# songxf1024/GIMS

Hardware: AMD Instinct MI355X
Metric: image-pairs/sec at 2x4096 keypoints (higher is better)
Workload: dtype bf16 MFMA attention + bf16x3 MFMA linears + f32 Sinkhorn; 1 GPU; 8 pairs/step/GPU of 2x4096 synthetic keypoints (kept 4096/4096 after AGC r=15 p=2 m=7), 256-d descriptors, 18 attentional layers (9 self + 9 cross), 100 Sinkhorn iterations, match_threshold 0.2; keypoints=4096

## Files before the change

gims_amd/csrc/agc.hip:

```cpp
#include "common.h"

#include <cstring>
#include <vector>

namespace gims {

constexpr int AGC_MAX_N = 32768;
constexpr int AGC_PK_SHIFT = 16;
constexpr uint32_t AGC_PK_MASK = 0xffffu;
constexpr int AGC_CC_LDS_N = 16384;
constexpr int AGC_NB = 16384;

struct AgcWs {
  float* dnf;
  uint16_t* dn16;
  uint16_t* S16;
  uint32_t* list;
  uint32_t* band;
  uint32_t* clist;
  uint32_t* ckey;
  uint32_t list_cap, clist_cap; int lds16;
  int32_t* cellptr;
  int32_t* cellidx;
  uint64_t* bits;
// ... 905 lines not shown
  extern __shared__ int32_t sm[];
  int32_t* list = sm;
  uint32_t* touched = (uint32_t*)(sm + w.n);
  __shared__ int wcount[17];
  const int t = threadIdx.x, lane = t & 63, wave = t >> 6;
  const int total_dir = w.counters[0];
  for (int k = t; k < (w.n + 31) / 32; k += 1024) touched[k] = 0;
  if (t == 0) wcount[16] = 0;
  __syncthreads();
  int n_added = 0;
  if (total_dir != 0 && w.n > 1) {
    for (int base = 0; base < w.n; base += 1024) {
      const int i = base + t;
      const bool iso = i < w.n && w.deg[i] == 0;
      const uint64_t m = __ballot(iso);
      if (lane == 0) wcount[wave] = __popcll(m);
      __syncthreads();
      int off = wcount[16];
      for (int q = 0; q < wave; ++q) off += wcount[q];
      if (iso) list[off + __popcll(m & ((1ull << lane) - 1))] = i;
      __syncthreads();
      if (t == 0) {
        int s = 0;
        for (int q = 0; q < 16; ++q) s += wcount[q];
        wcount[16] += s;
      }
      __syncthreads();
    }
    if (t == 0) {
      const int cnt = wcount[16];
      for (int q = 0; q < cnt; ++q) {
        const int i = list[q];
        if (touched[i >> 5] & (1u << (i & 31))) continue;
        const int j = w.nn[i];
        w.bits[(int64_t)i * w.nw + (j >> 6)] |= 1ull << (j & 63);
        w.bits[(int64_t)j * w.nw + (i >> 6)] |= 1ull << (i & 63);
        touched[j >> 5] |= 1u << (j & 31);
        ++n_added;
      }
    }
  }
  if (t == 0) info[3] = n_added;
}

__global__ __launch_bounds__(1024) void agc_scan_kernel(const AgcWs* __restrict__ ws, int mode) {
  const AgcWs& w = ws[blockIdx.y];
  const int n = w.n;
  const int32_t* deg = mode == 0 ? w.deg : (mode == 1 ? w.coff : w.degk);
  int32_t* ptr = mode == 0 ? w.ptr0 : (mode == 1 ? w.coff2 : w.indptr);
  int32_t* total_out = mode == 0 ? w.counters + 2 : (mode == 1 ? nullptr : w.info + 1);
  __shared__ int wsum[16];
  __shared__ int carry;
  const int t = threadIdx.x, lane = t & 63, wave = t >> 6;
  if (t == 0) carry = 0;
  __syncthreads();
  for (int base = 0; base < n; base += 1024) {
    const int i = base + t;
    int v = i < n ? deg[i] : 0;
    int x = v;
#pragma unroll
    for (int o = 1; o < 64; o <<= 1) {
      const int y = __shfl_up(x, o, 64);
      if (lane >= o) x += y;
    }
    if (lane == 63) wsum[wave] = x;
    __syncthreads();
    int off = carry;
    for (int q = 0; q < wave; ++q) off += wsum[q];
    if (i < n) ptr[i] = off + x - v;
    __syncthreads();
    if (t == 0) {
      int s = 0;
      for (int q = 0; q < 16; ++q) s += wsum[q];
      carry += s;
    }
    __syncthreads();
  }
  if (t == 0) {
    ptr[n] = carry;
    if (total_out) *total_out = carry;
  }
}

__global__ __launch_bounds__(256) void agc_fill_kernel(const AgcWs* __restrict__ ws, int final_pass) {
  const AgcWs& w = ws[blockIdx.y];
  const int32_t* __restrict__ ptr_by_row = final_pass ? w.indptr : w.ptr0;
  const int32_t* __restrict__ newid = final_pass ? w.newid : nullptr;
  int32_t* __restrict__ idx = final_pass ? w.indices : w.idx0;
  const int cap = final_pass ? w.max_edges_dir : w.cap;
  const int wave = threadIdx.x >> 6, lane = threadIdx.x & 63, sub = lane & 15;
  const int i = blockIdx.x * 16 + wave * 4 + (lane >> 4);
  const bool live = i < w.n && !(newid && newid[i] < 0);
  const int wpl = (w.nw + 15) / 16, k0 = sub * wpl, k1 = k0 + wpl < w.nw ? k0 + wpl : w.nw;
  int c = 0;
  if (live)
    for (int k = k0; k < k1; ++k) c += __popcll(w.bits[(int64_t)i * w.nw + k]);
  int x = c;
#pragma unroll
  for (int o = 1; o < 16; o <<= 1) {
    const int y = __shfl_up(x, o, 16);
    if (sub >= o) x += y;
  }
  if (!live) return;
  int pos = ptr_by_row[newid ? newid[i] : i] + x - c;
  for (int k = k0; k < k1; ++k) {
    uint64_t m = w.bits[(int64_t)i * w.nw + k];
    while (m) {
      const int b = __ffsll((unsigned long long)m) - 1;
      m &= m - 1;
      const int j = k * 64 + b;
      if (pos < cap) {
        idx[pos] = newid ? newid[j] : j;
        if (!final_pass) w.esrc[pos] = i;
      }
      ++pos;
    }
  }
}

template <bool GLOBAL>
__global__ __launch_bounds__(1024) void agc_cc_kernel(const AgcWs* __restrict__ ws) {
  const AgcWs& w = ws[blockIdx.y];
  const int min_size = w.min_size;
  int32_t* __restrict__ kept = w.kept;
  int32_t* info = w.info;
  extern __shared__ int32_t sm[];
  int32_t* parent = GLOBAL ? w.members : sm;
  int32_t* count = GLOBAL ? w.nnc : sm + w.n;
  auto cnt_of = [&](int x) { return __hip_atomic_load(&count[x], __ATOMIC_RELAXED, __HIP_MEMORY_SCOPE_AGENT); };
  __shared__ int wsum[16];
  __shared__ int carry[2];
  const int t = threadIdx.x, lane = t & 63, wave = t >> 6;
  const int n = w.n;
  for (int u = t; u < n; u += 1024) {
    __hip_atomic_store(&parent[u], u, __ATOMIC_RELAXED, __HIP_MEMORY_SCOPE_AGENT);
    __hip_atomic_store(&count[u], 0, __ATOMIC_RELAXED, __HIP_MEMORY_SCOPE_AGENT);
  }
  __syncthreads();
  volatile int32_t* vp = parent;
  auto find = [&](int x) {
    for (;;) {
      const int p = vp[x];
      if (p == x) return x;
      const int g = vp[p];
      if (g != p) vp[x] = g;
      x = p;
    }
  };
  {
    const int E = w.ptr0[n] < w.cap ? w.ptr0[n] : w.cap;
    for (int e0 = t; e0 < E; e0 += 4 * 1024) {
      int us[4], vs[4];
#pragma unroll
      for (int q = 0; q < 4; ++q) {
        const int e = e0 + q * 1024;
        us[q] = e < E ? w.esrc[e] : 0;
        vs[q] = e < E ? w.idx0[e] : 0;
      }
#pragma unroll
      for (int q = 0; q < 4; ++q) {
        const int u = us[q], v = vs[q];
        if (v <= u) continue;
        for (;;) {
          const int ru = find(u), rv = find(v);
          if (ru == rv) break;
          const int hi = ru > rv ? ru : rv, lo = ru > rv ? rv : ru;
          if (atomicCAS(&parent[hi], hi, lo) == hi) break;
        }
// ... 120 lines not shown
  const int C = w.counters[1];
  if (c >= C) return;
  const double cx = w.cent[2 * c], cy = w.cent[2 * c + 1];
  double bd = 1e300;
  int bj = 0x7fffffff;
  for (int j = lane; j < C; j += 64) {
    if (j == c) continue;
    const double dx = w.cent[2 * j] - cx, dy = w.cent[2 * j + 1] - cy;
    const double dd = dx * dx + dy * dy;
    if (dd < bd) { bd = dd; bj = j; }
  }
#pragma unroll
  for (int o = 32; o > 0; o >>= 1) {
    const double od = __shfl_xor(bd, o, 64);
    const int oj = __shfl_xor(bj, o, 64);
    if (od < bd || (od == bd && oj < bj)) { bd = od; bj = oj; }
  }
  if (lane == 0) w.nnc[c] = bj;
}

__global__ __launch_bounds__(256) void agc_link_kernel(const AgcWs* __restrict__ ws) {
  const AgcWs& w = ws[blockIdx.y];
  const float* __restrict__ kpts = w.kpts;
  const int32_t* __restrict__ coff = w.coff2;
  __shared__ double sd[256];
  __shared__ int sv[256], su[256];
  const int t = threadIdx.x;
  const int C = w.counters[1];
  if (C <= 1) return;
  for (int i = blockIdx.x; i < C; i += gridDim.x) {
  const int j = w.nnc[i];
  if (j < i && w.nnc[j] == i) {
    if (t == 0) { w.link[2 * i] = -1; w.link[2 * i + 1] = -1; }
    continue;
  }
  const int ai = coff[i], na = coff[i + 1] - ai;
  const int aj = coff[j], nb = coff[j + 1] - aj;
  double bd = 1e300;
  int bv = 0x7fffffff, bu = 0x7fffffff;
  const bool swap = nb > na;
  const int big0 = swap ? aj : ai, nbig = swap ? nb : na, small0 = swap ? ai : aj, nsmall = swap ? na : nb;
  for (int p = t; p < nbig; p += 256) {
    const int pb = w.members[big0 + p];
    const double bx = (double)kpts[2 * pb], by = (double)kpts[2 * pb + 1];
    for (int q = 0; q < nsmall; ++q) {
      const int ps = w.members[small0 + q];
      const double dx = bx - (double)kpts[2 * ps], dy = by - (double)kpts[2 * ps + 1];
      const double dd = dx * dx + dy * dy;
      const int v = swap ? pb : ps, u = swap ? ps : pb;
      if (dd < bd || (dd == bd && (v < bv || (v == bv && u < bu)))) { bd = dd; bv = v; bu = u; }
    }
  }
  sd[t] = bd; sv[t] = bv; su[t] = bu;
  __syncthreads();
  for (int s = 128; s > 0; s >>= 1) {
    if (t < s) {
      const double od = sd[t + s];
      const int ov = sv[t + s], ou = su[t + s];
      if (od < sd[t] || (od == sd[t] && (ov < sv[t] || (ov == sv[t] && ou < su[t])))) { sd[t] = od; sv[t] = ov; su[t] = ou; }
    }
    __syncthreads();
  }
  if (t == 0) { w.link[2 * i] = su[0]; w.link[2 * i + 1] = sv[0]; }
  __syncthreads();
  }
}

__global__ __launch_bounds__(256) void agc_link_apply_kernel(const AgcWs* __restrict__ ws) {
  const AgcWs& w = ws[blockIdx.y];
  int32_t* info = w.info;
  const int C = w.counters[1];
  if (C <= 1) { if (threadIdx.x == 0 && blockIdx.x == 0) info[5] = 0; return; }
  int added = 0;
  for (int i = blockIdx.x * 256 + threadIdx.x; i < C; i += gridDim.x * 256) {
    const int u = w.link[2 * i], v = w.link[2 * i + 1];
    if (u < 0) continue;
    atomicOr((unsigned long long*)&w.bits[(int64_t)u * w.nw + (v >> 6)], 1ull << (v & 63));
    atomicOr((unsigned long long*)&w.bits[(int64_t)v * w.nw + (u >> 6)], 1ull << (u & 63));
    ++added;
  }
  if (added) atomicAdd(&info[5], added);
}

__global__ void agc_finish_kernel(const AgcWs* __restrict__ ws, int window) {
  const AgcWs& w = ws[blockIdx.y];
  int32_t* info = w.info;
  const int max_edges_dir = w.max_edges_dir;
  info[2] = w.counters[0] / 2;
  info[6] = (int32_t)__float_as_uint(key_f32(w.sel[0]));
  info[7] = (info[1] > max_edges_dir || w.counters[0] > w.cap || w.counters[2] > w.cap) ? 1 : 0;
  if ((uint32_t)w.counters[4] > w.clist_cap) {
    info[7] = 1;
    info[2] = w.counters[4];
  }
  if (window) {
    const float thr = key_f32(w.sel[0]), vL = __uint_as_float(w.band[0]), vU = __uint_as_float(w.band[1]), eps = __uint_as_float(w.band[2]);
    if (w.counters[7] || !(thr >= vL + eps && thr <= vU - eps)) info[7] |= 2;
  } else {
    const float thr = key_f32(w.sel[0]);
    if (w.counters[7] || !(thr >= __uint_as_float(w.band[2]) && thr <= __uint_as_float(w.band[3]))) info[7] |= 2;
  }
}

__global__ __launch_bounds__(256) void agc_kept_deg_kernel(const AgcWs* __restrict__ ws) {
  const AgcWs& w = ws[blockIdx.y];
  const int u = blockIdx.x * 256 + threadIdx.x;
  if (u >= w.n) return;
  const int id = w.newid[u];
  if (id >= 0) w.degk[id] = w.deg[u];
  if (u >= w.info[0]) w.degk[u] = 0;
}

constexpr int AGC_MIN_CAP_PER_NODE = 64;

static void agc_layout(int n, int d, int max_edges_dir, bool with_s16, WsLayout& L, AgcWs& w) {
  const int nw = (n + 63) / 64, lds16 = (n + 7) & ~7;
  const int cap = max_edges_dir > n * AGC_MIN_CAP_PER_NODE ? max_edges_dir : n * AGC_MIN_CAP_PER_NODE;
  char* dn = L.take<char>((size_t)n * d * 6);
  w.dnf = (float*)dn;
  w.dn16 = dn ? (uint16_t*)(dn + (size_t)n * d * 4) : nullptr;
  const size_t list_cap = (size_t)n * (n - 1) / 2 + 64;
  w.S16 = with_s16 ? L.take<uint16_t>((size_t)n * lds16) : nullptr;
  w.clist = L.take<uint32_t>(cap);
  w.ckey = L.take<uint32_t>(cap);
  w.list = L.take<uint32_t>(list_cap);
  w.list_cap = (uint32_t)list_cap;
  w.clist_cap = (uint32_t)cap;
  w.lds16 = lds16;
  w.cellptr = L.take<int32_t>(AGC_NB + 1);
  w.cellidx = L.take<int32_t>(n);
  w.bits = L.take<uint64_t>((size_t)n * nw);
  w.hist = L.take<uint32_t>(4096);
  w.sel = L.take<uint32_t>(4);
  w.band = L.take<uint32_t>(4);
  w.deg = L.take<int32_t>(n);
  w.nn = L.take<int32_t>(n);
  w.label = L.take<int32_t>(n);
  w.alive = L.take<int32_t>(n);
  w.newid = L.take<int32_t>(n);
  w.crank = L.take<int32_t>(n);
  w.coff = L.take<int32_t>(n + 1);
  w.members = L.take<int32_t>(n);
  w.nnc = L.take<int32_t>(n);
  w.link = L.take<int32_t>((size_t)n * 2);
  w.cent = L.take<double>((size_t)n * 2);
  w.ptr0 = L.take<int32_t>(n + 1);
  w.idx0 = L.take<int32_t>(cap);
  w.esrc = L.take<int32_t>(cap);
  w.counters = L.take<int32_t>(16);
  w.coff2 = L.take<int32_t>(n + 1);
  w.degk = L.take<int32_t>(n);
  w.n = n; w.d = d; w.nw = nw; w.cap = cap;
}

static void agc_batch_layout(const gims_agc_image* images, int n_images, bool robust, WsLayout& L, AgcWs* recs) {
  L.take<AgcWs>(n_images);
  AgcWs scratch;
  for (int i = 0; i < n_images; ++i) agc_layout(images[i].n, images[i].d, images[i].max_edges_dir, robust, L, recs ? recs[i] : scratch);
}

}

static bool agc_takes_robust_flow(const gims_agc_image* images, int n_images, int flags) {
  bool robust = (flags & GIMS_AGC_ROBUST) != 0 || gims::env_int("GIMS_AGC_ROBUST", 0) != 0;
  for (int i = 0; i < n_images; ++i) robust = robust || images[i].d % gims::SW_KC != 0 || images[i].d > gims::SW_KMAX;
  return robust;
}

extern "C" size_t gims_agc_workspace_bytes(const gims_agc_image* images, int32_t n_images, int32_t flags) {
  using namespace gims;
  if (!images || n_images <= 0) return 0;
  const bool robust = agc_takes_robust_flow(images, n_images, flags);
  WsLayout L(nullptr);
  agc_batch_layout(images, n_images, robust, L, nullptr);
  return L.bytes();
}

extern "C" int32_t gims_agc_max_keypoints(void) { return gims::AGC_MAX_N; }

extern "C" int gims_agc_build(const gims_agc_image* images, int32_t n_images, const gims_agc_params* params, int32_t n_params, int32_t flags,
                              void* work, size_t work_bytes, void* stream) {
  using namespace gims;
  GIMS_CHECK_ARG(images && n_images > 0 && work, "gims_agc_build: null / empty arguments");
  GIMS_CHECK_ARG(params && (n_params == 1 || n_params == n_images), "gims_agc_build: h_params is null or n_params=%d is neither 1 nor n_images=%d",
                 n_params, n_images);
  const bool robust = agc_takes_robust_flow(images, n_images, flags);
  const char* env_shift = getenv("GIMS_AGC_WINDOW_SHIFT");
  const float window_test_shift = env_shift ? (float)atof(env_shift) : 0.f;
  for (int i = 0; i < n_images; ++i) {
    const gims_agc_image& im = images[i];
    GIMS_CHECK_ARG(im.kpts && im.desc && im.kept && im.indptr && im.indices && im.info, "gims_agc_build: image %d has a null pointer", i);
    GIMS_CHECK_ARG(im.n >= 2 && im.n <= AGC_MAX_N, "gims_agc_build: image %d: n=%d out of range [2, %d] (gims_agc_max_keypoints)", i, im.n, AGC_MAX_N);
    static_assert(AGC_MAX_N <= (1 << AGC_PK_SHIFT), "the band list packs a pair as i << 16 | j");
    GIMS_CHECK_ARG(im.d > 0 && (im.d % 32) == 0 && (im.ldd % 4) == 0, "gims_agc_build: image %d: d=%d must be a multiple of 32 (ldd %% 4 == 0)", i, im.d);
  }
  std::vector<AgcWs> hws(n_images);
  WsLayout lay(work);
  agc_batch_layout(images, n_images, robust, lay, hws.data());
  GIMS_CHECK_ARG(work_bytes >= lay.bytes(), "gims_agc_build: workspace too small (%zu bytes; gims_agc_workspace_bytes asks for %zu for the %s flow)", work_bytes,
                 lay.bytes(), robust ? "robust" : "window");
  hipStream_t s = (hipStream_t)stream;
  AgcWs* dws = (AgcWs*)work;
  int maxn = 0, maxnw = 0;
  for (int i = 0; i < n_images; ++i) {
    const gims_agc_image& im = images[i];
    AgcWs* w = &hws[i];
    w->kpts = im.kpts; w->desc = im.desc; w->ldd = im.ldd; w->kept = im.kept; w->indptr = im.indptr; w->indices = im.indices;
    w->info = im.info; w->max_edges_dir = im.max_edges_dir;
    const gims_agc_params& pm = params[n_params == 1 ? 0 : i];
    const int64_t L = (int64_t)im.n * (im.n - 1) / 2;
    int64_t k = (int64_t)(((double)L * pm.percentile) / 100.0);
    if (k >= L) k = L - 1;
    if (k < 0) k = 0;
    w->krank = k;
    double side = fabs(pm.radius) * 1.001;
    if (!(side >= 1e-3)) side = 1e-3;
    w->r2 = pm.radius * pm.radius;
    w->inv_side = 1.0 / side;
    w->min_size = pm.min_size;
    maxn = im.n > maxn ? im.n : maxn;
    maxnw = w->nw > maxnw ? w->nw : maxnw;
  }
  GIMS_LDS_ATTR((const void*)agc_cc_kernel<false>, AGC_CC_LDS_N * 8);
  GIMS_LDS_ATTR((const void*)agc_iso_seq_kernel, AGC_MAX_N * 4 + (AGC_MAX_N / 32 + 2) * 4);
  const int B = n_images;
  {
    const int rc = upload_table(hws.data(), sizeof(AgcWs) * (size_t)B, dws, s);
    if (rc != GIMS_OK) return rc;
    hipLaunchKernelGGL(agc_init_kernel, dim3(1, B), dim3(256), 0, s, dws);
  }
  const dim3 gw(cdiv(maxn, 4), B), g1(1, B);
  hipLaunchKernelGGL(agc_normalize_kernel, gw, dim3(256), 0, s, dws);
  {
    const int T = cdiv(maxn, S16_T), ntiles = T * (T + 1) / 2;
    if (robust) {
      GIMS_LDS_ATTR((const void*)agc_sim16_kernel, S16_LDS_BYTES);
      const int nparts = 8 / (((B & -B) > 8) ? 8 : (B & -B)), per_xcd = cdiv(B * nparts, 8) * cdiv(ntiles, nparts);
      const int sgrid = 8 * (per_xcd < 2 * (device_cus() / 8) ? per_xcd : 2 * (device_cus() / 8));
      int hgrid = 4096 / B;
      hgrid = hgrid < 16 ? 16 : (hgrid > 1024 ? 1024 : hgrid);
      hgrid = hgrid < maxn ? hgrid : maxn;
      hipLaunchKernelGGL(agc_sim16_kernel, dim3(sgrid), dim3(256), S16_LDS_BYTES, s, dws, B);
      hipLaunchKernelGGL(agc_band_kernel, g1, dim3(256), 0, s, dws);
      hipLaunchKernelGGL(agc_sweep16_kernel, dim3(hgrid, B), dim3(256), 0, s, dws, 1);
    } else {
      GIMS_LDS_ATTR((const void*)agc_simw_kernel<SIM_SAMPLE>, SW_LDS_BYTES);
      GIMS_LDS_ATTR((const void*)agc_simw_kernel<SIM_COLLECT>, SW_LDS_BYTES);
      const int wgrid = 8 * 2 * (device_cus() / 8);
      hipLaunchKernelGGL(agc_simw_kernel<SIM_SAMPLE>, dim3(wgrid), dim3(256), SW_LDS_BYTES, s, dws, B);
      hipLaunchKernelGGL(agc_window_kernel, g1, dim3(256), 0, s, dws, window_test_shift);
      hipLaunchKernelGGL(agc_simw_kernel<SIM_COLLECT>, dim3(wgrid), dim3(256), SW_LDS_BYTES, s, dws, B);
    }
    GIMS_LDS_ATTR((const void*)agc_grid_kernel, AGC_NB * 4);
    hipLaunchKernelGGL(agc_grid_kernel, g1, dim3(1024), AGC_NB * 4, s, dws);
    hipLaunchKernelGGL(agc_radius_grid_kernel, dim3(cdiv(maxn, 32), B), dim3(288), 0, s, dws);
    hipLaunchKernelGGL(agc_exact_kernel, dim3(8 * 4 * (device_cus() / 8)), dim3(256), 0, s, dws, B, robust ? 0 : 1);
    const int lgrid = 1024 / B < 4 ? 4 : (1024 / B > 64 ? 64 : 1024 / B);
    hipLaunchKernelGGL(agc_hist_kernel, dim3(lgrid, B), dim3(256), 0, s, dws, 20, 12);
    hipLaunchKernelGGL(agc_pick_kernel, g1, dim3(256), 0, s, dws, 20, 12);
    hipLaunchKernelGGL(agc_hist_kernel, dim3(lgrid, B), dim3(256), 0, s, dws, 8, 12);
    hipLaunchKernelGGL(agc_pick_kernel, g1, dim3(256), 0, s, dws, 8, 12);
    hipLaunchKernelGGL(agc_hist_kernel, dim3(lgrid, B), dim3(256), 0, s, dws, 0, 8);
    hipLaunchKernelGGL(agc_pick_kernel, g1, dim3(256), 0, s, dws, 0, 8);
  }
  hipLaunchKernelGGL(agc_apply_kernel, dim3(16, B), dim3(256), 0, s, dws);
  hipLaunchKernelGGL(agc_deg_kernel, dim3(cdiv(maxn, 16), B), dim3(256), 0, s, dws, 1);
  hipLaunchKernelGGL(agc_iso_nn_kernel, gw, dim3(256), 0, s, dws);
  const size_t iso_lds = (size_t)maxn * 4 + ((size_t)(maxn + 31) / 32 + 1) * 4;
  hipLaunchKernelGGL(agc_iso_seq_kernel, g1, dim3(1024), iso_lds, s, dws);
  hipLaunchKernelGGL(agc_deg_kernel, dim3(cdiv(maxn, 16), B), dim3(256), 0, s, dws, 0);
  hipLaunchKernelGGL(agc_scan_kernel, g1, dim3(1024), 0, s, dws, 0);
  hipLaunchKernelGGL(agc_fill_kernel, dim3(cdiv(maxn, 16), B), dim3(256), 0, s, dws, 0);
  if (maxn <= AGC_CC_LDS_N) hipLaunchKernelGGL(agc_cc_kernel<false>, g1, dim3(1024), (size_t)maxn * 8, s, dws);
  else hipLaunchKernelGGL(agc_cc_kernel<true>, g1, dim3(1024), 0, s, dws);
  hipLaunchKernelGGL(agc_scan_kernel, g1, dim3(1024), 0, s, dws, 1);
  if (maxn <= 16384) hipLaunchKernelGGL(agc_members_kernel<4>, dim3(32, B), dim3(256), 0, s, dws);
  else hipLaunchKernelGGL(agc_members_kernel<8>, dim3(32, B), dim3(512), 0, s, dws);
  hipLaunchKernelGGL(agc_nnc_kernel, gw, dim3(256), 0, s, dws);
  hipLaunchKernelGGL(agc_link_kernel, dim3(maxn < 256 ? maxn : 256, B), dim3(256), 0, s, dws);
  hipLaunchKernelGGL(agc_link_apply_kernel, dim3(cdiv(maxn, 256), B), dim3(256), 0, s, dws);
  hipLaunchKernelGGL(agc_deg_kernel, dim3(cdiv(maxn, 16), B), dim3(256), 0, s, dws, 0);
  hipLaunchKernelGGL(agc_kept_deg_kernel, dim3(cdiv(maxn, 256), B), dim3(256), 0, s, dws);
  hipLaunchKernelGGL(agc_scan_kernel, g1, dim3(1024), 0, s, dws, 2);
  hipLaunchKernelGGL(agc_fill_kernel, dim3(cdiv(maxn, 16), B), dim3(256), 0, s, dws, 1);
  hipLaunchKernelGGL(agc_finish_kernel, g1, dim3(1), 0, s, dws, robust ? 0 : 1);
  GIMS_LAUNCH_CHECK();
  return GIMS_OK;
}
```

gims_amd/csrc/common.h:

```cpp
#pragma once
#include <hip/hip_runtime.h>
#include <stdint.h>
#include <stdio.h>
#include <stdlib.h>

#include "../../include/gims_hip.h"

namespace gims {

void set_error(const char* fmt, ...);

#define GIMS_CHECK_ARG(cond, ...)                    \
  do {                                               \
    if (!(cond)) {                                   \
      ::gims::set_error(__VA_ARGS__);                \
      return GIMS_EINVAL;                            \
    }                                                \
  } while (0)

#define GIMS_HIP(call)                                                                     \
  do {                                                                                     \
    hipError_t e_ = (call);                                                                \
    if (e_ != hipSuccess) {                                                                \
      ::gims::set_error("%s failed: %s (%s:%d)", #call, hipGetErrorString(e_), __FILE__, __LINE__); \
// ... 48 lines not shown
#pragma unroll
  for (int o = 32; o > 0; o >>= 1) v = fmaxf(v, __shfl_xor(v, o, 64));
  return v;
}
__device__ __forceinline__ double wave_sum_f64(double v) {
#pragma unroll
  for (int o = 32; o > 0; o >>= 1) v += __shfl_xor(v, o, 64);
  return v;
}

__device__ __forceinline__ uint32_t f32_key(float x) {
  uint32_t u = __float_as_uint(x);
  return (u & 0x80000000u) ? ~u : (u | 0x80000000u);
}
__device__ __forceinline__ float key_f32(uint32_t k) {
  uint32_t u = (k & 0x80000000u) ? (k & 0x7fffffffu) : ~k;
  return __uint_as_float(u);
}

__device__ __forceinline__ void ot_raise_status(float* status, float code) {
  __hip_atomic_fetch_max((int*)status, __float_as_int(code), __ATOMIC_RELAXED, __HIP_MEMORY_SCOPE_AGENT);
}

__device__ __forceinline__ bool attn_guard_fires(const gims_attn_guard& g) {
  const unsigned long long* st = (const unsigned long long*)g.stat;
  const int lane = threadIdx.x & 63, nw = 4 * (g.n_heads + 1);
  const unsigned long long v = lane < nw ? __builtin_nontemporal_load(st + lane) : 0ull;
  bool mine = false;
  if (g.kind == GIMS_GUARD_PEAKED) {
    const unsigned long long cnt = __shfl(v, (lane & ~3) + 1, 64), tail = __shfl(v, (lane & ~3) + 3, 64);
    const unsigned long long mx = __shfl(v, (lane & ~3) + 2, 64);
    if ((lane & 3) == 0 && lane < 4 * g.n_heads) {
      if (cnt != 0) {
        const double mean = (double)v / (double)cnt / 16777216.0, tl = (double)tail / (double)cnt;
        mine = mean > g.mean_thr || tl > g.tail_thr;
      }
      mine = mine || (g.max_thr > 0.0 && (double)mx / 16777216.0 >= g.max_thr);
    }
  } else if (lane >= 4 * g.n_heads && lane < 4 * g.n_heads + 3) {
    mine = !((double)__uint_as_float((uint32_t)v) <= g.range_limit);
  }
  return __ballot(mine) != 0ull;
}

static inline int cdiv(int64_t a, int64_t b) { return (int)((a + b - 1) / b); }

static inline size_t al256(size_t x) { return (x + 255) & ~(size_t)255; }
struct WsLayout {
  char* base;
  size_t off = 0;
  explicit WsLayout(void* b) : base((char*)b) {}
  template <typename T> T* take(size_t count) { const size_t o = off; off += al256(sizeof(T) * count); return base ? (T*)(base + o) : nullptr; }
  size_t bytes() const { return off; }
};
static inline int env_int(const char* name, int dflt) { const char* e = getenv(name); return e ? atoi(e) : dflt; }
static inline bool guard_walk_enabled() { return env_int("GIMS_GUARD_WALK", 1) != 0; }

int upload_table(const void* host, size_t bytes, void* dev, hipStream_t stream);
int lds_attr(const void* fn, int bytes);
void* device_once(const char* key, size_t bytes, const void* init);
void* pinned_once(const char* key, size_t bytes);
int current_device();
int device_cus();
void count_linear_launch(int kind);
int linear_x6_batch_launch(const gims_linear_args* dev_args, int count, int max_m, int max_n, hipStream_t s);
int split_spl3_launch(const float* src, int64_t lds, uint16_t* dst, int64_t ldd, int64_t rows, int k, hipStream_t s);

int mlp_fused_launch(const gims_linear_args& a, hipStream_t s);

int sift_describe_aux(const gims_aux_args& x, hipStream_t st);
int diou_nms_aux(const gims_aux_args& x, hipStream_t st);
int assemble_rows_aux(const gims_aux_args& x, hipStream_t st);
int build_tracks_aux(const gims_aux_args& x, hipStream_t st);
int triangulate_tracks_aux(const gims_aux_args& x, hipStream_t st);
int resect_images_aux(const gims_aux_args& x, hipStream_t st);
int bundle_adjust_aux(const gims_aux_args& x, hipStream_t st);
int bundle_adjust_pcg_aux(const gims_aux_args& x, hipStream_t st);
int bundle_adjust_focal_aux(const gims_aux_args& x, hipStream_t st);
int select_pairs_aux(const gims_aux_args& x, hipStream_t st);

struct OtR2Host { const float* z; int64_t ld; int n, m; float* u; float* v; float* status; float norm, log_mu_bin, log_nu_bin; };
struct OtR2Plan { bool ok; int nx, nc, ppg, ngroups; size_t bytes; };
OtR2Plan ot_res2_plan(const OtR2Host* pr, int np, int iters);
int ot_res2_run(const OtR2Plan& P, const OtR2Host* hp, int np, float alpha, int iters, int init_inside, char* base, hipStream_t s);

}
```

gims_amd/csrc/misc.hip:

```cpp
#include "common.h"

#include <stdarg.h>
#include <string.h>

#include <map>
#include <mutex>
#include <string>
#include <utility>

namespace gims {

static thread_local char g_err[512] = "";
void set_error(const char* fmt, ...) {
  va_list ap;
  va_start(ap, fmt);
  vsnprintf(g_err, sizeof(g_err), fmt, ap);
  va_end(ap);
}

int current_device() {
  int dev = 0;
  if (hipGetDevice(&dev) != hipSuccess) dev = 0;
  return dev;
}

int device_cus() {
  int n = 0;
  if (hipDeviceGetAttribute(&n, hipDeviceAttributeMultiprocessorCount, current_device()) != hipSuccess || n < 8) n = 8;
  return n;
}

static std::mutex g_once_mu;

int lds_attr(const void* fn, int bytes) {
  static std::map<std::pair<const void*, int>, int> done;
  const int dev = current_device();
  std::lock_guard<std::mutex> lock(g_once_mu);
  int& have = done[std::make_pair(fn, dev)];
  if (have >= bytes) return GIMS_OK;
  GIMS_HIP(hipFuncSetAttribute(fn, hipFuncAttributeMaxDynamicSharedMemorySize, bytes));
  have = bytes;
  return GIMS_OK;
}

void* device_once(const char* key, size_t bytes, const void* init) {
  static std::map<std::pair<std::string, int>, void*> bufs;
  const int dev = current_device();
  std::lock_guard<std::mutex> lock(g_once_mu);
  void*& p = bufs[std::make_pair(std::string(key), dev)];
  if (p) return p;
  void* d = nullptr;
  if (hipMalloc(&d, bytes) != hipSuccess) return nullptr;
  if ((init ? hipMemcpy(d, init, bytes, hipMemcpyHostToDevice) : hipMemset(d, 0, bytes)) != hipSuccess) { (void)hipFree(d); return nullptr; }
  p = d;
  return p;
}

void* pinned_once(const char* key, size_t bytes) {
  static std::map<std::pair<std::string, int>, void*> bufs;
  const int dev = current_device();
  std::lock_guard<std::mutex> lock(g_once_mu);
  void*& p = bufs[std::make_pair(std::string(key), dev)];
  if (p) return p;
  void* h = nullptr;
  if (hipHostMalloc(&h, bytes) != hipSuccess) return nullptr;
  memset(h, 0, bytes);
  p = h;
  return p;
}

struct Blob4K { uint4 v[248]; };
__global__ void put_blob_kernel(Blob4K blob, uint4* __restrict__ dst, int n16) {
  if ((int)threadIdx.x < n16) dst[threadIdx.x] = blob.v[threadIdx.x];
}

int upload_table(const void* host, size_t bytes, void* dev, hipStream_t stream) {
  const char* h = (const char*)host;
  char* d = (char*)dev;
  for (size_t off = 0; off < bytes; off += sizeof(Blob4K)) {
    Blob4K blob;
    const size_t n = bytes - off < sizeof(Blob4K) ? bytes - off : sizeof(Blob4K);
    memcpy(&blob, h + off, n);
    hipLaunchKernelGGL(put_blob_kernel, dim3(1), dim3(256), 0, stream, blob, (uint4*)(d + off), (int)((n + 15) / 16));
  }
  GIMS_LAUNCH_CHECK();
  return GIMS_OK;
}

}

extern "C" int gims_upload_table(const void* host, int64_t bytes, void* dev, void* stream) {
  using namespace gims;
  GIMS_CHECK_ARG(host && dev && bytes >= 0 && bytes <= (1 << 20) && ((uintptr_t)dev & 15) == 0, "gims_upload_table: bad arguments");
  if (bytes == 0) return GIMS_OK;
  return upload_table(host, (size_t)bytes, dev, (hipStream_t)stream);
}

namespace gims {
template <bool RELU>
__global__ __launch_bounds__(256) void kenc_first_kernel(const float* __restrict__ kpts, const float* __restrict__ norm3,
                                                         const int32_t* __restrict__ seg, const float* __restrict__ w1,
                                                         const float* __restrict__ b1, int c1, float* __restrict__ out,
                                                         int64_t n, int n_img) {
  const int64_t idx = (int64_t)blockIdx.x * blockDim.x + threadIdx.x;
  const int64_t row = idx / c1;
  const int ch = (int)(idx - row * c1);
  if (row >= n) return;
  int img;
  if (n_img > 0) {
    int lo = 0, hi = n_img - 1;
    while (lo < hi) {
      const int mid = (lo + hi + 1) >> 1;
      if ((int64_t)seg[mid] <= row) lo = mid; else hi = mid - 1;
    }
    img = lo;
  } else {
    img = seg[row];
  }
  const float* nm = norm3 + 3 * img;
  const float x = (kpts[2 * row] - nm[0]) / nm[2];
  const float y = (kpts[2 * row + 1] - nm[1]) / nm[2];
  float v = fmaf(w1[2 * ch + 1], y, fmaf(w1[2 * ch], x, b1[ch]));
  out[row * c1 + ch] = RELU ? fmaxf(v, 0.f) : v;
}

__global__ __launch_bounds__(256) void layernorm_act_kernel(const float* __restrict__ x, int64_t ldx, int64_t rows, int c,
                                                            const float* __restrict__ a2, const float* __restrict__ b2, float eps, int act,
                                                            float* __restrict__ out, int64_t ldo, uint16_t* __restrict__ out_hi,
                                                            uint16_t* __restrict__ out_lo, int64_t ld_split) {
  const int64_t row = (int64_t)blockIdx.x * 4 + (threadIdx.x >> 6);
  const int lane = threadIdx.x & 63;
  if (row >= rows) return;
  const float* xr = x + row * ldx;
  float v[8];
  float s = 0.f;
#pragma unroll
  for (int k = 0; k < 8; ++k) {
    const int ch = lane + 64 * k;
    v[k] = ch < c ? xr[ch] : 0.f;
    s += v[k];
  }
  const float mean = wave_sum(s) / (float)c;
  float q = 0.f;
#pragma unroll
  for (int k = 0; k < 8; ++k) {
    const float d = lane + 64 * k < c ? v[k] - mean : 0.f;
    q += d * d;
  }
  const float sd = sqrtf(wave_sum(q) / (float)(c - 1));
  const float inv = 1.f / (sd + eps);
#pragma unroll
  for (int k = 0; k < 8; ++k) {
    const int ch = lane + 64 * k;
    if (ch < c) {
      float y = a2[ch] * ((v[k] - mean) * inv) + b2[ch];
      if (act == GIMS_ACT_RELU) y = fmaxf(y, 0.f);
      if (out) out[row * ldo + ch] = y;
      if (out_hi) {
        const uint16_t h = f2bf(y);
        out_hi[row * ld_split + spl_col(ch)] = h;
        out_lo[row * ld_split + spl_col(ch)] = f2bf(y - bf2f(h));
      }
    }
  }
}

__global__ __launch_bounds__(256) void sage_mean_kernel(const float* __restrict__ h, int64_t ldh,
                                                        const int32_t* __restrict__ indptr,
                                                        const int32_t* __restrict__ indices, int n, int c,
                                                        float* __restrict__ out, int64_t ldo,
                                                        uint16_t* __restrict__ out_spl, int64_t ld_spl) {
  const int wave = threadIdx.x >> 6, lane = threadIdx.x & 63;
  const int node = blockIdx.x * 4 + wave;
  if (node >= n) return;
  const int beg = indptr[node], end = indptr[node + 1];
  for (int q0 = 0; 4 * q0 < c; q0 += 64) {
    const int q = q0 + lane;
    const bool act = 4 * q < c;
    const int qq = act ? q : 0;
    float4 s = make_float4(0.f, 0.f, 0.f, 0.f);
    for (int e0 = beg; e0 < end; e0 += 64) {
      const int cnt = end - e0 < 64 ? end - e0 : 64;
      const int mine = lane < cnt ? indices[e0 + lane] : 0;
      int e = 0;
      for (; e + 4 <= cnt; e += 4) {
        const float4 x0 = *(const float4*)(h + (int64_t)__shfl(mine, e, 64) * ldh + 4 * qq);
        const float4 x1 = *(const float4*)(h + (int64_t)__shfl(mine, e + 1, 64) * ldh + 4 * qq);
        const float4 x2 = *(const float4*)(h + (int64_t)__shfl(mine, e + 2, 64) * ldh + 4 * qq);
        const float4 x3 = *(const float4*)(h + (int64_t)__shfl(mine, e + 3, 64) * ldh + 4 * qq);
        s.x += x0.x; s.y += x0.y; s.z += x0.z; s.w += x0.w;
        s.x += x1.x; s.y += x1.y; s.z += x1.z; s.w += x1.w;
        s.x += x2.x; s.y += x2.y; s.z += x2.z; s.w += x2.w;
        s.x += x3.x; s.y += x3.y; s.z += x3.z; s.w += x3.w;
      }
      for (; e < cnt; ++e) {
        const float4 x = *(const float4*)(h + (int64_t)__shfl(mine, e, 64) * ldh + 4 * qq);
        s.x += x.x; s.y += x.y; s.z += x.z; s.w += x.w;
      }
    }
    if (!act) continue;
    if (end > beg) {
      const float d = (float)(end - beg);
      s.x /= d; s.y /= d; s.z /= d; s.w /= d;
    }
    if (out) *(float4*)(out + (int64_t)node * ldo + 4 * q) = s;
    if (out_spl) {
      const uint32_t h01 = pack_bf2(s.x, s.y), h23 = pack_bf2(s.z, s.w);
      const uint32_t l01 = pack_bf2(s.x - __uint_as_float(h01 << 16), s.y - __uint_as_float(h01 & 0xffff0000u));
      const uint32_t l23 = pack_bf2(s.z - __uint_as_float(h23 << 16), s.w - __uint_as_float(h23 & 0xffff0000u));
      uint16_t* o = out_spl + (int64_t)node * ld_spl + spl_col(4 * q);
      *(uint2*)o = make_uint2(h01, h23);
      *(uint2*)(o + 32) = make_uint2(l01, l23);
    }
  }
}

__global__ __launch_bounds__(256) void gather_rows_kernel(const float* __restrict__ src, int64_t lds,
                                                          const int32_t* __restrict__ idx, int n, int c,
                                                          float* __restrict__ dst, int64_t ldd) {
  const int wave = threadIdx.x >> 6, lane = threadIdx.x & 63;
  const int row = blockIdx.x * 4 + wave;
  if (row >= n) return;
  const float* s = src + (int64_t)idx[row] * lds;
  float* d = dst + (int64_t)row * ldd;
  for (int j = lane; j < c; j += 64) d[j] = s[j];
}

__global__ __launch_bounds__(256) void pack_graphs_kernel(const gims_pack_image* __restrict__ imgs, int d,
                                                          float* __restrict__ feat, int64_t ldf,
                                                          float* __restrict__ kpts_out, float* __restrict__ score_out,
                                                          int32_t* __restrict__ seg, int32_t* __restrict__ indptr_out,
                                                          int32_t* __restrict__ indices_out, int n_rows_total,
                                                          int n_edges_total) {
  const gims_pack_image im = imgs[blockIdx.y];
  const int wave = threadIdx.x >> 6, lane = threadIdx.x & 63;
  for (int r = blockIdx.x * 4 + wave; r < im.n_kept; r += gridDim.x * 4) {
    const int src = im.kept[r];
    const float4* s = (const float4*)(im.desc + (int64_t)src * im.ldd);
    float4* o = (float4*)(feat + (int64_t)(im.row_off + r) * ldf);
    for (int q = lane; 4 * q < d; q += 64) o[q] = s[q];
    if (lane == 0) {
      kpts_out[2 * (im.row_off + r)] = im.kpts[2 * src];
      kpts_out[2 * (im.row_off + r) + 1] = im.kpts[2 * src + 1];
      if (score_out && im.score) score_out[im.row_off + r] = im.score[src];
      seg[im.row_off + r] = blockIdx.y;
      if (im.src_row) im.src_row[im.row_off + r] = im.in_off + src;
      indptr_out[im.row_off + r] = im.indptr[r] + im.edge_off;
    }
  }
  for (int e = blockIdx.x * 256 + threadIdx.x; e < im.n_edges; e += gridDim.x * 256)
    indices_out[im.edge_off + e] = im.indices[e] + im.row_off;
  if (blockIdx.x == 0 && blockIdx.y == 0 && threadIdx.x == 0) indptr_out[n_rows_total] = n_edges_total;
}

__global__ __launch_bounds__(256) void ingest_kernel(const gims_ingest_image* __restrict__ imgs, int d,
                                                     float* __restrict__ desc_out, int64_t ldo,
                                                     float* __restrict__ kpts_out, float* __restrict__ score_out) {
  __shared__ float tile[64][65];
  const gims_ingest_image im = imgs[blockIdx.z];
  const int n0 = blockIdx.x * 64, d0 = blockIdx.y * 64;
  if (n0 >= im.n) return;
  const int c = threadIdx.x & 63, r4 = threadIdx.x >> 6;
#pragma unroll
  for (int i = 0; i < 16; ++i) {
    const int r = 4 * i + r4;
    const int n = n0 + c;
    tile[r][c] = (d0 + r < d && n < im.n) ? im.desc[(int64_t)(d0 + r) * im.ldd + n] : 0.f;
  }
  __syncthreads();
#pragma unroll
  for (int i = 0; i < 16; ++i) {
    const int r = 4 * i + r4;
    const int n = n0 + r;
    if (n < im.n && d0 + c < d) desc_out[(int64_t)(im.row_off + n) * ldo + d0 + c] = tile[c][r];
  }
  if (blockIdx.y == 0 && threadIdx.x < 64) {
    const int n = n0 + threadIdx.x;
    if (n < im.n) {
      kpts_out[2 * (im.row_off + n)] = im.kpts[2 * n];
      kpts_out[2 * (im.row_off + n) + 1] = im.kpts[2 * n + 1];
      if (score_out) score_out[im.row_off + n] = im.score ? im.score[n] : 0.f;
    }
  }
}

}

extern "C" int gims_ingest_images(const gims_ingest_image* dev_images, int32_t n_images, int32_t max_n, int32_t d,
                                  float* desc_out, int64_t ldo, float* kpts_out, float* score_out, void* stream) {
  using namespace gims;
  GIMS_CHECK_ARG(dev_images && n_images > 0 && max_n > 0 && d > 0 && desc_out && kpts_out, "gims_ingest_images: bad arguments");
  hipLaunchKernelGGL(ingest_kernel, dim3(cdiv(max_n, 64), cdiv(d, 64), n_images), dim3(256), 0, (hipStream_t)stream,
                     dev_images, d, desc_out, ldo, kpts_out, score_out);
  GIMS_LAUNCH_CHECK();
  return GIMS_OK;
}

extern "C" int gims_pack_graphs(const gims_pack_image* dev_images, int32_t n_images, int32_t max_kept, int32_t max_edges,
                                int32_t d, float* feat, int64_t ldf, float* kpts_out, float* score_out, int32_t* seg,
                                int32_t* indptr_out, int32_t* indices_out, int32_t n_rows_total, int32_t n_edges_total,
                                void* stream) {
  using namespace gims;
  GIMS_CHECK_ARG(dev_images && n_images > 0 && feat && kpts_out && seg && indptr_out && indices_out, "gims_pack_graphs: null pointer");
  GIMS_CHECK_ARG((d % 4) == 0 && (ldf % 4) == 0, "gims_pack_graphs: d / ldf must be multiples of 4");
  int gx = cdiv(max_kept, 4);
  const int ge = cdiv(max_edges, 256);
  gx = gx > ge ? gx : ge;
  if (gx < 1) gx = 1;
  if (gx > 1024) gx = 1024;
  hipLaunchKernelGGL(pack_graphs_kernel, dim3(gx, n_images), dim3(256), 0, (hipStream_t)stream, dev_images, d, feat, ldf,
                     kpts_out, score_out, seg, indptr_out, indices_out, n_rows_total, n_edges_total);
  GIMS_LAUNCH_CHECK();
  return GIMS_OK;
}

static int kenc_first_images(const float* kpts, const float* norm3, const int32_t* starts, const float* w1, const float* b1, int32_t c1,
                             float* out, int64_t n, int32_t n_img, hipStream_t stream) {
  using namespace gims;
  GIMS_CHECK_ARG(kpts && norm3 && starts && w1 && b1 && out && c1 > 0 && n >= 0, "gims_run_ops: GIMS_AUX_KENC_FIRST: bad arguments");
  if (n == 0) return GIMS_OK;
  hipLaunchKernelGGL(kenc_first_kernel<true>, dim3(cdiv(n * c1, 256)), dim3(256), 0, stream, kpts, norm3, starts, w1, b1, c1, out, n, n_img);
  GIMS_LAUNCH_CHECK();
  return GIMS_OK;
}

extern "C" int gims_run_ops(const gims_op* ops, int32_t n_ops, void* stream) {
  using namespace gims;
  GIMS_CHECK_ARG(ops && n_ops >= 0, "gims_run_ops: bad arguments");
  for (int i = 0; i < n_ops; ++i) {
    int rc;
    if (ops[i].kind == GIMS_OP_LINEAR) {
      rc = gims_linear(&ops[i].u.lin, stream);
    } else if (ops[i].kind == GIMS_OP_ATTENTION) {
      rc = gims_attention(&ops[i].u.att, stream);
    } else if (ops[i].kind == GIMS_OP_MLP) {
      rc = mlp_fused_launch(ops[i].u.lin, (hipStream_t)stream);
    } else if (ops[i].kind == GIMS_OP_AUX) {
      const gims_aux_args& x = ops[i].u.aux;
      if (x.fn == GIMS_AUX_SPLIT_SPL32)
        rc = gims_split_spl32((const float*)x.p[0], x.i[0], (uint16_t*)x.p[1], x.i[1], x.i[2], (int32_t)x.i[3], stream);
      else if (x.fn == GIMS_AUX_SAGE_MEAN_SPLIT)
        rc = gims_sage_mean_split((const float*)x.p[0], x.i[0], (const int32_t*)x.p[1], (const int32_t*)x.p[2], (int32_t)x.i[1], (int32_t)x.i[2],
                                  (uint16_t*)x.p[3], x.i[3], stream);
      else if (x.fn == GIMS_AUX_KENC_FIRST && x.i[2] > 0)
        rc = kenc_first_images((const float*)x.p[0], (const float*)x.p[1], (const int32_t*)x.p[2], (const float*)x.p[3], (const float*)x.p[4],
                               (int32_t)x.i[0], (float*)x.p[5], x.i[1], (int32_t)x.i[2], (hipStream_t)stream);
      else if (x.fn == GIMS_AUX_KENC_FIRST)
        rc = gims_kenc_first((const float*)x.p[0], (const float*)x.p[1], (const int32_t*)x.p[2], (const float*)x.p[3], (const float*)x.p[4],
                             (int32_t)x.i[0], (float*)x.p[5], x.i[1], stream);
      else if (x.fn == GIMS_AUX_SAGE_MEAN)
        rc = gims_sage_mean((const float*)x.p[0], x.i[0], (const int32_t*)x.p[1], (const int32_t*)x.p[2], (int32_t)x.i[1], (int32_t)x.i[2],
                            (float*)x.p[3], x.i[3], stream);
      else if (x.fn == GIMS_AUX_KENC_FIRST_LINEAR)
        rc = gims_kenc_first_linear((const float*)x.p[0], (const float*)x.p[1], (const int32_t*)x.p[2], (const float*)x.p[3], (const float*)x.p[4],
                                    (int32_t)x.i[0], (float*)x.p[5], x.i[1], stream);
      else if (x.fn == GIMS_AUX_LAYERNORM_ACT)
        rc = gims_layernorm_act((const float*)x.p[0], x.i[0], x.i[1], (int32_t)x.i[2], (const float*)x.p[1], (const float*)x.p[2], x.f[0], (int32_t)x.i[3],
                                (float*)x.p[3], x.i[4], (uint16_t*)x.p[4], (uint16_t*)x.p[5], x.i[5], stream);
      else if (x.fn == GIMS_AUX_SIFT_DESCRIBE)
        rc = sift_describe_aux(x, (hipStream_t)stream);
      else if (x.fn == GIMS_AUX_DIOU_NMS)
        rc = diou_nms_aux(x, (hipStream_t)stream);
      else if (x.fn == GIMS_AUX_ASSEMBLE_ROWS)
        rc = assemble_rows_aux(x, (hipStream_t)stream);
      else if (x.fn == GIMS_AUX_BUILD_TRACKS)
        rc = build_tracks_aux(x, (hipStream_t)stream);
      else if (x.fn == GIMS_AUX_TRIANGULATE_TRACKS)
        rc = triangulate_tracks_aux(x, (hipStream_t)stream);
      else if (x.fn == GIMS_AUX_RESECT_IMAGES)
        rc = resect_images_aux(x, (hipStream_t)stream);
      else if (x.fn == GIMS_AUX_BUNDLE_ADJUST)
        rc = bundle_adjust_aux(x, (hipStream_t)stream);
      else if (x.fn == GIMS_AUX_BUNDLE_ADJUST_PCG)
        rc = bundle_adjust_pcg_aux(x, (hipStream_t)stream);
      else if (x.fn == GIMS_AUX_BUNDLE_ADJUST_FOCAL)
        rc = bundle_adjust_focal_aux(x, (hipStream_t)stream);
      else if (x.fn == GIMS_AUX_SELECT_PAIRS)
        rc = select_pairs_aux(x, (hipStream_t)stream);
      else
        GIMS_CHECK_ARG(false, "gims_run_ops: op %d: unknown auxiliary function %d", i, x.fn);
    } else {
      GIMS_CHECK_ARG(false, "gims_run_ops: op %d has unknown kind %d", i, ops[i].kind);
    }
    if (rc != GIMS_OK) return rc;
  }
  return GIMS_OK;
}

extern "C" int gims_run_ops_timed(const gims_op* ops, int32_t n_ops, void* stream, void* const* events) {
  using namespace gims;
  GIMS_CHECK_ARG(ops && n_ops >= 0 && events, "gims_run_ops_timed: bad arguments");
  GIMS_HIP(hipEventRecord((hipEvent_t)events[0], (hipStream_t)stream));
  for (int i = 0; i < n_ops; ++i) {
    const int rc = gims_run_ops(ops + i, 1, stream);
    if (rc != GIMS_OK) return rc;
    GIMS_HIP(hipEventRecord((hipEvent_t)events[i + 1], (hipStream_t)stream));
  }
  return GIMS_OK;
}

extern "C" int gims_events_create(int32_t n, void** events_out) {
  using namespace gims;
  GIMS_CHECK_ARG(n > 0 && events_out, "gims_events_create: bad arguments");
  for (int i = 0; i < n; ++i) {
    hipEvent_t e = nullptr;
    const hipError_t rc = hipEventCreate(&e);
    if (rc != hipSuccess) {
      for (int j = 0; j < i; ++j) (void)hipEventDestroy((hipEvent_t)events_out[j]);
      GIMS_HIP(rc);
    }
    events_out[i] = (void*)e;
  }
  return GIMS_OK;
}

extern "C" int gims_events_elapsed(void* const* events, int32_t n, float* ms_out) {
  using namespace gims;
  GIMS_CHECK_ARG(events && n > 1 && ms_out, "gims_events_elapsed: bad arguments");
  for (int i = 0; i + 1 < n; ++i) GIMS_HIP(hipEventElapsedTime(&ms_out[i], (hipEvent_t)events[i], (hipEvent_t)events[i + 1]));
  return GIMS_OK;
}

extern "C" int gims_events_destroy(void* const* events, int32_t n) {
  using namespace gims;
  GIMS_CHECK_ARG(events && n >= 0, "gims_events_destroy: bad arguments");
  for (int i = 0; i < n; ++i)
    if (events[i]) GIMS_HIP(hipEventDestroy((hipEvent_t)events[i]));
  return GIMS_OK;
}

extern "C" int gims_ops_graph_create(const gims_op* ops, int32_t n_ops, void* stream, void** graph_exec_out) {
  using namespace gims;
  GIMS_CHECK_ARG(ops && n_ops > 0 && graph_exec_out && stream, "gims_ops_graph_create: bad arguments (a non-default stream is required)");
  hipStream_t s = (hipStream_t)stream;
  GIMS_HIP(hipStreamBeginCapture(s, hipStreamCaptureModeThreadLocal));
  const int rc = gims_run_ops(ops, n_ops, stream);
  hipGraph_t graph = nullptr;
  const hipError_t e = hipStreamEndCapture(s, &graph);
  if (rc != GIMS_OK) { if (graph) (void)hipGraphDestroy(graph); return rc; }
  GIMS_HIP(e);
  hipGraphExec_t exec = nullptr;
  const hipError_t e2 = hipGraphInstantiate(&exec, graph, nullptr, nullptr, 0);
  (void)hipGraphDestroy(graph);
  GIMS_HIP(e2);
  *graph_exec_out = (void*)exec;
  return GIMS_OK;
}

extern "C" int gims_ops_graph_launch(void* graph_exec, void* stream) {
  using namespace gims;
  GIMS_CHECK_ARG(graph_exec, "gims_ops_graph_launch: null graph");
  GIMS_HIP(hipGraphLaunch((hipGraphExec_t)graph_exec, (hipStream_t)stream));
  return GIMS_OK;
}

extern "C" int gims_ops_graph_destroy(void* graph_exec) {
  using namespace gims;
  if (graph_exec) GIMS_HIP(hipGraphExecDestroy((hipGraphExec_t)graph_exec));
  return GIMS_OK;
}

extern "C" int gims_abi_version(void) { return GIMS_ABI_VERSION; }
extern "C" const char* gims_last_error(void) { return gims::g_err; }

extern "C" int gims_kenc_first(const float* kpts, const float* norm3, const int32_t* seg_of_row, const float* w1,
                               const float* b1, int32_t c1, float* out, int64_t n, void* stream) {
  using namespace gims;
  GIMS_CHECK_ARG(kpts && norm3 && seg_of_row && w1 && b1 && out && c1 > 0 && n >= 0, "gims_kenc_first: bad arguments");
  if (n == 0) return GIMS_OK;
  hipLaunchKernelGGL(kenc_first_kernel<true>, dim3(cdiv(n * c1, 256)), dim3(256), 0, (hipStream_t)stream, kpts, norm3,
                     seg_of_row, w1, b1, c1, out, n, 0);
  GIMS_LAUNCH_CHECK();
  return GIMS_OK;
}

extern "C" int gims_kenc_first_linear(const float* kpts, const float* norm3, const int32_t* seg_of_row, const float* w1,
                                      const float* b1, int32_t c1, float* out, int64_t n, void* stream) {
  using namespace gims;
  GIMS_CHECK_ARG(kpts && norm3 && seg_of_row && w1 && b1 && out && c1 > 0 && n >= 0, "gims_kenc_first_linear: bad arguments");
  if (n == 0) return GIMS_OK;
  hipLaunchKernelGGL(kenc_first_kernel<false>, dim3(cdiv(n * c1, 256)), dim3(256), 0, (hipStream_t)stream, kpts, norm3,
                     seg_of_row, w1, b1, c1, out, n, 0);
  GIMS_LAUNCH_CHECK();
  return GIMS_OK;
}

extern "C" int gims_layernorm_act(const float* x, int64_t ldx, int64_t rows, int32_t c, const float* a2, const float* b2, float eps,
                                  int32_t act, float* out, int64_t ldo, uint16_t* out_hi, uint16_t* out_lo, int64_t ld_split,
                                  void* stream) {
  using namespace gims;
  GIMS_CHECK_ARG(x && a2 && b2 && (out || out_hi) && rows >= 0 && c >= 2 && c <= 512, "gims_layernorm_act: bad arguments (2 <= c <= 512)");
  GIMS_CHECK_ARG((out_hi == nullptr) == (out_lo == nullptr), "gims_layernorm_act: out_hi and out_lo come together");
  GIMS_CHECK_ARG(ldx >= c && (!out || ldo >= c) && (!out_hi || ld_split >= 2 * (int64_t)((c + 31) / 32 * 32)),
                 "gims_layernorm_act: pitch below the row width (ldx, ldo >= c; SPL32 pitch >= 2 * c rounded up to 32 channels)");
  if (rows == 0) return GIMS_OK;
  hipLaunchKernelGGL(layernorm_act_kernel, dim3((unsigned)cdiv(rows, 4)), dim3(256), 0, (hipStream_t)stream, x, ldx, rows, c, a2, b2, eps,
                     act, out, ldo, out_hi, out_lo, ld_split);
  GIMS_LAUNCH_CHECK();
  return GIMS_OK;
}

extern "C" int gims_sage_mean(const float* h, int64_t ldh, const int32_t* indptr, const int32_t* indices, int32_t n,
                              int32_t c, float* out, int64_t ldo, void* stream) {
  using namespace gims;
  GIMS_CHECK_ARG(h && indptr && indices && out && n >= 0, "gims_sage_mean: bad arguments");
  GIMS_CHECK_ARG((c % 4) == 0 && (ldh % 4) == 0 && (ldo % 4) == 0, "gims_sage_mean: c / ld must be multiples of 4");
  if (n == 0) return GIMS_OK;
  hipLaunchKernelGGL(sage_mean_kernel, dim3(cdiv(n, 4)), dim3(256), 0, (hipStream_t)stream, h, ldh, indptr, indices, n, c,
                     out, ldo, (uint16_t*)nullptr, (int64_t)0);
  GIMS_LAUNCH_CHECK();
  return GIMS_OK;
}

extern "C" int gims_sage_mean_split(const float* h, int64_t ldh, const int32_t* indptr, const int32_t* indices, int32_t n,
                                    int32_t c, uint16_t* out_spl, int64_t ld_spl, void* stream) {
  using namespace gims;
  GIMS_CHECK_ARG(h && indptr && indices && out_spl && n >= 0, "gims_sage_mean_split: bad arguments");
  GIMS_CHECK_ARG((c % 4) == 0 && (ldh % 4) == 0 && (ld_spl % 4) == 0 && ld_spl >= 2 * (int64_t)((c + 31) / 32 * 32) && ((uintptr_t)out_spl & 7) == 0,
                 "gims_sage_mean_split: c / ldh multiples of 4, SPL32 output pitch >= 2 * c rounded up to 32 channels");
  if (n == 0) return GIMS_OK;
  hipLaunchKernelGGL(sage_mean_kernel, dim3(cdiv(n, 4)), dim3(256), 0, (hipStream_t)stream, h, ldh, indptr, indices, n, c,
                     (float*)nullptr, (int64_t)0, out_spl, ld_spl);
  GIMS_LAUNCH_CHECK();
  return GIMS_OK;
}

__global__ __launch_bounds__(256) void pair_stats_kernel(const int64_t* __restrict__ matches0, const float* __restrict__ scores0,
                                                         const int32_t* __restrict__ tab, float* __restrict__ out) {
  const int p = blockIdx.x, t = threadIdx.x;
  const int n0 = tab[4 * p + 1], off = tab[4 * p + 3];
  __shared__ float ssum[256];
  __shared__ int scnt[256];
  float s = 0.f;
  int c = 0;
  for (int i = t; i < n0; i += 256)
    if (matches0[off + i] >= 0) { s += scores0[off + i]; ++c; }
  ssum[t] = s;
  scnt[t] = c;
  __syncthreads();
  for (int o = 128; o > 0; o >>= 1) {
    if (t < o) { ssum[t] += ssum[t + o]; scnt[t] += scnt[t + o]; }
    __syncthreads();
  }
  if (t == 0) {
    float* r = out + 5 * p;
    r[0] = (float)tab[4 * p]; r[1] = (float)n0; r[2] = (float)tab[4 * p + 2];
    r[3] = (float)scnt[0]; r[4] = ssum[0] / fmaxf((float)scnt[0], 1.f);
  }
}

extern "C" int gims_pair_stats(const int64_t* matches0, const float* scores0, const int32_t* table, int32_t n_pairs, float* out,
                               void* stream) {
  using namespace gims;
  GIMS_CHECK_ARG(matches0 && scores0 && table && out && n_pairs >= 0, "gims_pair_stats: bad arguments");
  if (n_pairs == 0) return GIMS_OK;
  hipLaunchKernelGGL(pair_stats_kernel, dim3(n_pairs), dim3(256), 0, (hipStream_t)stream, matches0, scores0, table, out);
  GIMS_LAUNCH_CHECK();
  return GIMS_OK;
}

extern "C" int gims_gather_rows(const float* src, int64_t lds, const int32_t* idx, int32_t n, int32_t c, float* dst,
                                int64_t ldd, void* stream) {
  using namespace gims;
  GIMS_CHECK_ARG(src && idx && dst && n >= 0 && c > 0, "gims_gather_rows: bad arguments");
  GIMS_CHECK_ARG(lds >= c && ldd >= c, "gims_gather_rows: pitch below the row width");
// ... 6 lines not shown
```

gims_amd/csrc/sinkhorn.hip:

```cpp
#include "common.h"

#include <stdio.h>
#include <stdlib.h>
#include <string.h>

#include <map>
#include <mutex>
#include <type_traits>
#include <vector>

namespace gims {

constexpr int OT_R = 8;

struct OtDev {
  const float* z; int64_t ld; int n, m;
  float* u; float* v;
  float* partial;
  float* cbest_val; int* cbest_idx;
  float* max0; int* idx0;
  float* max1; int* idx1;
  int64_t* matches0; int64_t* matches1; float* mscores0; float* mscores1;
  float* status;
  int G;
// ... 1023 lines not shown
  const int rows = ot_instance(cpt, [](auto inst) { return decltype(inst)::R; });
  const int total = threads >= 1024 ? 256 : (threads >= 512 ? 512 : 1024);
  int cap = total / (np > 0 ? np : 1);
  if (cap < 4) cap = 4;
  int g = (n + rows - 1) / rows;
  return g < cap ? g : cap;
}
static void ot_fill_common(const gims_ot_problem& q, float& norm, float& log_mu_bin, float& log_nu_bin) {
  const float ms = (float)q.n, ns = (float)q.m;
  norm = -logf(ms + ns);
  log_mu_bin = logf(ns) + norm;
  log_nu_bin = logf(ms) + norm;
}

struct OtWs { int threads, cpt, maxn, maxm, maxG; OtR2Plan plan2; char* onchip; };
static OtWs ot_layout(const gims_ot_problem* pr, int np, int flags, WsLayout& L, OtDev* recs) {
  OtWs w{};
  ot_launch_shape(pr, np, w.threads, w.cpt, w.maxn, w.maxm);
  L.take<OtDev>(np);
  for (int i = 0; i < np; ++i) {
    const gims_ot_problem& q = pr[i];
    OtDev d{};
    d.G = ot_G(q.n, np, w.threads, w.cpt);
    w.maxG = d.G > w.maxG ? d.G : w.maxG;
    d.partial = L.take<float>((size_t)d.G * (q.m + 1));
    d.cbest_val = L.take<float>((size_t)d.G * q.m);
    d.cbest_idx = L.take<int>((size_t)d.G * q.m);
    d.max0 = L.take<float>(q.n);
    d.idx0 = L.take<int>(q.n);
    d.max1 = L.take<float>(q.m);
    d.idx1 = L.take<int>(q.m);
    if (!recs) continue;
    d.z = q.scores; d.ld = q.ld; d.n = q.n; d.m = q.m;
    d.u = q.uv; d.v = q.uv + q.n + 1; d.status = q.uv + q.n + 1 + q.m + 1;
    d.matches0 = q.matches0; d.matches1 = q.matches1; d.mscores0 = q.mscores0; d.mscores1 = q.mscores1;
    ot_fill_common(q, d.norm, d.log_mu_bin, d.log_nu_bin);
    recs[i] = d;
  }
  w.plan2 = ot_res2_choose(pr, np, 1, flags);
  w.onchip = L.take<char>(w.plan2.bytes);
  return w;
}

static void ot_streamed_iteration(const OtWs& w, const OtDev* dp, int np, float alpha, int rescue, int hist_slot, hipStream_t s) {
  const dim3 gi(w.maxG, np), gc(cdiv(w.maxm + 1, 64), np), bt(w.threads);
  ot_instance(w.cpt, [&](auto inst) { using I = decltype(inst); hipLaunchKernelGGL((ot_iter_kernel<I::CPT, I::R>), gi, bt, 0, s, dp, alpha, rescue); });
  hipLaunchKernelGGL(ot_colreduce_kernel, gc, dim3(1024), 0, s, dp, hist_slot, rescue);
}

}

extern "C" int gims_sinkhorn_plan(const gims_ot_problem* pr, int32_t np, int32_t iters, int32_t flags) {
  using namespace gims;
  if (!pr || np <= 0) return 0;
  const OtR2Plan p2 = ot_res2_choose(pr, np, iters, flags);
  return p2.ok ? p2.ngroups : 0;
}

extern "C" int gims_sinkhorn_match(const gims_ot_problem* pr, int32_t np, float alpha, int32_t iters, float match_threshold, void* work,
                                   size_t work_bytes, int32_t flags, void* stream) {
  using namespace gims;
  hipStream_t s = (hipStream_t)stream;
  GIMS_CHECK_ARG(pr && np > 0 && work, "gims_sinkhorn_match: null / empty arguments");
  GIMS_CHECK_ARG(iters >= 0, "gims_sinkhorn_match: iters < 0");
  for (int i = 0; i < np; ++i) {
    const gims_ot_problem& q = pr[i];
    GIMS_CHECK_ARG(q.n > 0 && q.m > 0 && q.scores && q.uv && q.matches0 && q.matches1 && q.mscores0 && q.mscores1,
                   "gims_sinkhorn_match: problem %d has empty shape or null pointer", i);
    GIMS_CHECK_ARG((q.ld % 4) == 0 && (((uintptr_t)q.scores) & 15) == 0, "gims_sinkhorn_match: scores must be 16-byte aligned with ld %% 4 == 0");
  }
  std::vector<OtDev> hprob(np);
  WsLayout L(work);
  const OtWs w = ot_layout(pr, np, flags, L, hprob.data());
  GIMS_CHECK_ARG(work_bytes >= L.bytes(), "gims_sinkhorn_match: workspace too small (%zu < %zu)", work_bytes, L.bytes());
  GIMS_CHECK_ARG(w.cpt <= 8, "gims_sinkhorn_match: m=%d too large (max 32768 columns: a thread of the streamed kernels owns at most 8 column quads)", w.maxm);
  const int threads = w.threads, cpt = w.cpt, maxn = w.maxn, maxm = w.maxm;
  {
    const int rc = upload_table(hprob.data(), sizeof(OtDev) * (size_t)np, work, s);
    if (rc != GIMS_OK) return rc;
  }
  const OtDev* dp = (const OtDev*)work;
  const bool onchip = w.plan2.ok && iters >= 1;
  const int init_inside = onchip && env_int("GIMS_OT_R2_INIT", 1) ? 1 : 0;
  if (init_inside) hipLaunchKernelGGL(ot_status0_kernel, dim3(cdiv(np, 256)), dim3(256), 0, s, dp, np);
  else hipLaunchKernelGGL(ot_init_kernel, dim3(cdiv(maxn, 4), np), dim3(256), 0, s, dp, alpha, iters == 0 ? 1 : 0, 0);
  const dim3 gi(w.maxG, np);
  if (onchip) {
    std::vector<OtR2Host> h2(np);
    for (int i = 0; i < np; ++i) {
      const OtDev& d = hprob[i];
      h2[i] = OtR2Host{d.z, d.ld, d.n, d.m, d.u, d.v, d.status, d.norm, d.log_mu_bin, d.log_nu_bin};
    }
    const int rc = ot_res2_run(w.plan2, h2.data(), np, alpha, iters, init_inside, w.onchip, s);
    if (rc != GIMS_OK) return rc;
    const int force_fail = env_int("GIMS_OT_FORCE_FAIL", 0);
    if (force_fail) hipLaunchKernelGGL(ot_poison_kernel, dim3(np), dim3(256), 0, s, dp);
    OtRescueState* rs = ot_rescue_state();
    if (!rs) { set_error("gims_sinkhorn_match: no rescue state on this device"); return GIMS_EHIP; }
    const int mode = env_int("GIMS_OT_RESCUE", -1);
    bool marginal;
    {
      std::lock_guard<std::mutex> lock(g_rescue_mu);
      rs->calls += 1;
      if (*rs->h_count != rs->seen) { rs->seen = *rs->h_count; rs->last_giveup_call = rs->calls; }
      marginal = mode == 1 || (mode != 0 && rs->calls - rs->last_giveup_call <= OT_MARGINAL_CALLS);
    }
    if (marginal) {
      hipLaunchKernelGGL(ot_rescue_begin_kernel, dim3(cdiv(np, 256)), dim3(256), 0, s, dp, np, rs->d_count);
      hipLaunchKernelGGL(ot_init_kernel, dim3(cdiv(maxn, 4), np), dim3(256), 0, s, dp, alpha, 0, 1);
      for (int it = 0; it < iters; ++it) ot_streamed_iteration(w, dp, np, alpha, 1, -1, s);
      hipLaunchKernelGGL(ot_rescue_end_kernel, dim3(cdiv(np, 256)), dim3(256), 0, s, dp, np);
    }
    hipLaunchKernelGGL(ot_rescue_kernel, dim3(np), dim3(1024), 0, s, dp, alpha, iters, 0, rs->d_count);
    if (hipEventQuery(rs->ev) != hipErrorNotReady) {
      GIMS_HIP(hipMemcpyAsync((void*)rs->h_count, rs->d_count, sizeof(int), hipMemcpyDeviceToHost, s));
      GIMS_HIP(hipEventRecord(rs->ev, s));
    }
  } else {
    for (int it = 0; it < iters; ++it) ot_streamed_iteration(w, dp, np, alpha, 0, -1, s);
  }
  ot_instance(cpt, [&](auto inst) { using I = decltype(inst); hipLaunchKernelGGL((ot_select_kernel<I::CPT, I::RS>), gi, dim3(threads), 0, s, dp); });
  hipLaunchKernelGGL(ot_colbest_kernel, dim3(cdiv(maxm, 32), np), dim3(256), 0, s, dp);
  const int mx = maxn > maxm ? maxn : maxm;
  hipLaunchKernelGGL(ot_mutual_kernel, dim3(cdiv(mx, 256), np), dim3(256), 0, s, dp, match_threshold);
  GIMS_LAUNCH_CHECK();
  return GIMS_OK;
}

extern "C" size_t gims_sinkhorn_workspace_bytes(const gims_ot_problem* pr, int32_t np) {
  using namespace gims;
  if (!pr || np <= 0) return 0;
  WsLayout L(nullptr);
  ot_layout(pr, np, 0, L, nullptr);
  return L.bytes();
}

extern "C" int64_t gims_sinkhorn_rescues(void) {
  using namespace gims;
  OtRescueState* rs = ot_rescue_state();
  int n = 0;
  if (!rs || hipDeviceSynchronize() != hipSuccess || hipMemcpy(&n, rs->d_count, sizeof(int), hipMemcpyDeviceToHost) != hipSuccess) {
    set_error("gims_sinkhorn_rescues: the counter of the current device could not be read");
    return -1;
  }
  return n;
}

extern "C" int gims_ot_matrix(const float* scores, int64_t ld, int32_t n, int32_t m, float alpha, const float* uv,
                              float* out, void* stream) {
  using namespace gims;
  GIMS_CHECK_ARG(scores && uv && out && n > 0 && m > 0, "gims_ot_matrix: bad arguments");
  hipLaunchKernelGGL(ot_matrix_kernel, dim3(cdiv(m + 1, 256), n + 1), dim3(256), 0, (hipStream_t)stream, scores, ld, n, m,
                     alpha, uv, out);
  GIMS_LAUNCH_CHECK();
  return GIMS_OK;
}

extern "C" int gims_train_loss(const gims_loss_pair* dev_pairs, int32_t n_pairs, const int64_t* gt, int32_t n_gt, float alpha,
                               float pos_weight, float neg_weight, float* loss_vec, int32_t* tag, float* out3, void* stream) {
  using namespace gims;
  GIMS_CHECK_ARG(dev_pairs && n_pairs > 0 && n_pairs <= 1024 && out3 && n_gt >= 0 && (n_gt == 0 || (gt && loss_vec && tag)),
                 "gims_train_loss: bad arguments (1 <= n_pairs <= 1024)");
  if (n_gt > 0) hipLaunchKernelGGL(train_loss_gather_kernel, dim3(cdiv(n_gt, 256)), dim3(256), 0, (hipStream_t)stream, dev_pairs, n_pairs, gt, n_gt, alpha,
                                   loss_vec, tag);
  hipLaunchKernelGGL(train_loss_reduce_kernel, dim3(1), dim3(1024), 0, (hipStream_t)stream, loss_vec, tag, n_gt, n_pairs, pos_weight, neg_weight, out3);
  GIMS_LAUNCH_CHECK();
  return GIMS_OK;
}

extern "C" size_t gims_sinkhorn_history_floats(int32_t n, int32_t m, int32_t iters) {
  return (size_t)(iters + 1) * (size_t)(n + m + 2);
}

extern "C" int gims_sinkhorn_history(const gims_ot_problem* pr, int32_t np, float alpha, int32_t iters, float* const* h_hist, void* work,
                                     size_t work_bytes, void* stream) {
  using namespace gims;
// ... 132 lines not shown
```

gims_amd/csrc/sinkhorn2d.hip:

```cpp
#include "common.h"

#include <stdlib.h>

#include <map>
#include <mutex>
#include <type_traits>
#include <vector>

namespace gims {

struct OtR2Block { int prob, xr, cc, pad; };
struct OtR2Dev {
  const float* z; int64_t ld; int n, m;
  float* u; float* v; float* status;
  float norm, log_mu_bin, log_nu_bin;
  float mu, mu_bin, nu_bin;
  int nx, nc;
  int rb, cb;
  int rbf, rbs;
  float* rpart;
  float* fbuf;
  float* cpart;
  float* mpart;
  int* placement;
  int* rflag;
};
struct OtR2Args {
  const OtR2Dev* probs;
  int p0, pcount, nx, nc;
  float alpha; int iters, refresh, wt_local;
  int init_inside;
  unsigned long long* prof;
};

constexpr int R2_FLAG_ITERS = 1024;
constexpr int R2_CSEG = 132;
constexpr int R2_NT = 512;
struct R2L {
  static constexpr int NW = R2_NT / 64;
  static constexpr int K = 16 * R2_NT * 4;
  static constexpr int NXMAX = 4;
  static constexpr int ROWST = 1028, FACS = 1160, GVEC = 132, COLRED = NW * 128, PB = 2 * R2_NT + 4, PR = 132, CSST = 132;
  static constexpr int XRD = 4 * R2_CSEG;
  static constexpr int OWN = 2 * 132 + 2 * 132;
  static constexpr int FLOATS = K + ROWST + FACS + GVEC + COLRED + PB + PR + CSST + XRD + 16 + OWN;
};

typedef float r2f2 __attribute__((ext_vector_type(2)));

__device__ __forceinline__ void r2_st4_wt(float* p, f32x4 v) { asm volatile("global_store_dwordx4 %0, %1, off sc1" ::"v"(p), "v"(v) : "memory"); }
__device__ __forceinline__ void r2_st4_plain(float* p, f32x4 v) { asm volatile("global_store_dwordx4 %0, %1, off" ::"v"(p), "v"(v) : "memory"); }
__device__ __forceinline__ void r2_ld4_issue(f32x4& v, const float* p) { asm volatile("global_load_dwordx4 %0, %1, off sc1" : "=&v"(v) : "v"(p) : "memory"); }
__device__ __forceinline__ void r2_ld4_wait(f32x4& a) { asm volatile("s_waitcnt vmcnt(0)" : "+v"(a)::"memory"); }
__device__ __forceinline__ void r2_swap16(float& x, float& y) { asm("s_nop 1\n\tv_permlane16_swap_b32 %0, %1" : "+v"(x), "+v"(y)); }
__device__ __forceinline__ void r2_swap32(float& x, float& y) { asm("s_nop 1\n\tv_permlane32_swap_b32 %0, %1" : "+v"(x), "+v"(y)); }
template <int CTRL>
__device__ __forceinline__ float r2_dpp_max(float x) {
  return fmaxf(x, __builtin_bit_cast(float, __builtin_amdgcn_update_dpp(0, __builtin_bit_cast(int, x), CTRL, 0xf, 0xf, true)));
}
template <int CTRL>
__device__ __forceinline__ float r2_dpp_add(float x) {
  return x + __builtin_bit_cast(float, __builtin_amdgcn_update_dpp(0, __builtin_bit_cast(int, x), CTRL, 0xf, 0xf, true));
}
__device__ __forceinline__ float r2_sum8(float x) {
  x = r2_dpp_add<0xB1>(x);
  x = r2_dpp_add<0x4E>(x);
  return r2_dpp_add<0x141>(x);
}

template <bool PROF>
__global__ __launch_bounds__(R2_NT, 1) void ot_res2_kernel(OtR2Args a) {
#pragma clang fp contract(off)
  using L = R2L;
  constexpr int NT = R2_NT;
  __shared__ int fail_flag;
  __shared__ unsigned long long prof_acc[8];
  unsigned long long prof_t = 0;
  auto stamp = [&](int phase) {
    if (PROF && threadIdx.x == 0) {
      const unsigned long long now = __builtin_readcyclecounter();
      if (phase >= 0) prof_acc[phase] += now - prof_t;
      prof_t = now;
    }
  };
  if (PROF && threadIdx.x < 8) prof_acc[threadIdx.x] = 0;
// ... 668 lines not shown
    float* rpart = L.take<float>((size_t)P.nx * P.nc * rbs);
    float* fbuf = L.take<float>((size_t)P.nx * 2 * rbs);
    float* cpart = L.take<float>((size_t)2 * P.nx * P.nc * R2_CSEG);
    float* mpart = L.take<float>((size_t)P.nx * P.nc * rbs);
    if (!recs) continue;
    const OtR2Host& d = pr[i];
    OtR2Dev q{};
    q.z = d.z; q.ld = d.ld; q.n = d.n; q.m = d.m; q.u = d.u; q.v = d.v; q.status = d.status;
    q.norm = d.norm; q.log_mu_bin = d.log_mu_bin; q.log_nu_bin = d.log_nu_bin;
    q.mu = (float)exp((double)d.norm); q.mu_bin = (float)exp((double)d.log_mu_bin); q.nu_bin = (float)exp((double)d.log_nu_bin);
    q.nx = P.nx; q.nc = P.nc; q.rb = rb; q.cb = r2_up4(cdiv(d.m, P.nc)); q.rbf = rbf; q.rbs = rbs;
    q.rpart = rpart; q.fbuf = fbuf; q.cpart = cpart; q.mpart = mpart;
    q.placement = w.dplace;
    recs[i] = q;
  }
  w.ex1 = L.bytes();
  for (int i = 0; i < np; ++i) {
    int* rflag = L.take<int>(R2_FLAG_ITERS + 8);
    if (recs) recs[i].rflag = rflag;
  }
  w.rf1 = L.bytes();
  L.take<OtR2Block>((size_t)512 * P.ngroups);
  return w;
}

static OtR2Plan plan_class(const OtR2Host* pr, int np, int iters) {
  OtR2Plan P{};
  if (iters < 1 || np < 1) return P;
  int nx = 0, nc = 0;
  if (!r2_geom(pr[0].n, pr[0].m, nx, nc)) return P;
  for (int i = 1; i < np; ++i) {
    int nxi = 0, nci = 0;
    if (!r2_geom(pr[i].n, pr[i].m, nxi, nci) || nxi != nx || nci != nc) return P;
  }
  const int units = 8 * (32 / nc);
  if (nx > units) return P;
  P.nx = nx; P.nc = nc;
  P.ppg = units / nx;
  P.ppg = P.ppg < np ? P.ppg : np;
  P.ngroups = cdiv(np, P.ppg);
  if (P.ngroups > 64) return P;
  for (int i = 0; i < np; ++i) {
    const int rb = cdiv(pr[i].n, nx);
    if (r2_up4(cdiv(rb + 1, nc)) > R2_FOLD || rb > r2_rbmax() || r2_up4(cdiv(pr[i].m, nc)) > 128) return P;
  }
  WsLayout L(nullptr);
  r2_layout(P, pr, np, L, nullptr);
  P.bytes = L.bytes();
  P.ok = true;
  return P;
}

static std::vector<std::vector<int>> r2_classes(const OtR2Host* pr, int np) {
  std::vector<std::vector<int>> out;
  std::vector<int> keys;
  for (int i = 0; i < np; ++i) {
    const int k = r2_class_key(pr[i]);
    size_t c = 0;
    while (c < keys.size() && keys[c] != k) ++c;
    if (c == keys.size()) { keys.push_back(k); out.emplace_back(); }
    out[c].push_back(i);
  }
  return out;
}

OtR2Plan ot_res2_plan(const OtR2Host* pr, int np, int iters) {
  OtR2Plan P{};
  if (iters < 1 || np < 1) return P;
  P.ok = true;
  for (const std::vector<int>& cls : r2_classes(pr, np)) {
    std::vector<OtR2Host> sub;
    for (int i : cls) sub.push_back(pr[i]);
    const OtR2Plan c = plan_class(sub.data(), (int)sub.size(), iters);
    if (!c.ok) return OtR2Plan{};
    P.nx = c.nx > P.nx ? c.nx : P.nx;
    P.nc = c.nc > P.nc ? c.nc : P.nc;
    P.ppg = c.ppg > P.ppg ? c.ppg : P.ppg;
    P.ngroups += c.ngroups;
    P.bytes += al256(c.bytes);
  }
  return P;
}

static int run_class(const OtR2Plan& P, const OtR2Host* hp, int np, float alpha, int iters, int init_inside, char* base, hipStream_t s);

struct R2State { int resident_ok, wt_local; volatile int* h_place; hipEvent_t place_ev; };
static R2State* r2_state(const void* kernel, int threads, int blocks, size_t lds) {
  static std::mutex mu;
  static std::map<int, R2State> states;
  const int dev = current_device();
  std::lock_guard<std::mutex> lock(mu);
  auto it = states.find(dev);
  if (it != states.end()) return &it->second;
  R2State st{};
  int per_cu = 0, cus = 0;
  const hipError_t e = hipOccupancyMaxActiveBlocksPerMultiprocessor(&per_cu, kernel, threads, lds);
  if (hipDeviceGetAttribute(&cus, hipDeviceAttributeMultiprocessorCount, dev) != hipSuccess) cus = 0;
  st.resident_ok = (e == hipSuccess && per_cu * cus >= blocks) ? 1 : 0;
  st.wt_local = env_int("GIMS_OT_R2_WT", 0) ? 1 : 0;
  st.h_place = (volatile int*)pinned_once("ot_res2_place", 256);
  if (!st.h_place || hipEventCreateWithFlags(&st.place_ev, hipEventDisableTiming) != hipSuccess) return nullptr;
  return &states.emplace(dev, st).first->second;
}

int ot_res2_run(const OtR2Plan&, const OtR2Host* hp, int np, float alpha, int iters, int init_inside, char* base, hipStream_t s) {
  WsLayout L(base);
  for (const std::vector<int>& cls : r2_classes(hp, np)) {
    std::vector<OtR2Host> sub;
    for (int i : cls) sub.push_back(hp[i]);
    const OtR2Plan c = plan_class(sub.data(), (int)sub.size(), iters);
    if (!c.ok) { set_error("ot_res2_run: a geometry class has no plan"); return GIMS_EINVAL; }
    const int rc = run_class(c, sub.data(), (int)sub.size(), alpha, iters, init_inside, L.take<char>(c.bytes), s);
    if (rc != GIMS_OK) return rc;
  }
  return GIMS_OK;
}

static int run_class(const OtR2Plan& P, const OtR2Host* hp, int np, float alpha, int iters, int init_inside, char* base, hipStream_t s) {
  std::vector<OtR2Dev> hd(np);
  WsLayout L(base);
  const R2Ws w = r2_layout(P, hp, np, L, hd.data());
  OtR2Dev* const dprob = w.dprob;
  int* const dplace = w.dplace;
  GIMS_HIP(hipMemsetAsync(base + w.ex0, 0xFF, w.ex1 - w.ex0, s));
  GIMS_HIP(hipMemsetAsync(base + w.ex1, 0, w.rf1 - w.ex1, s));
  GIMS_HIP(hipMemsetAsync(dplace, 0, 256, s));
  int rc = upload_table(hd.data(), sizeof(OtR2Dev) * (size_t)np, dprob, s);
  if (rc != GIMS_OK) return rc;
  const int nthreads = R2_NT, nblocks = 256;
  const size_t lds = R2L::FLOATS * sizeof(float);
  GIMS_LDS_ATTR((const void*)ot_res2_kernel<false>, (int)(R2L::FLOATS * sizeof(float)));
  GIMS_LDS_ATTR((const void*)ot_res2_kernel<true>, (int)(R2L::FLOATS * sizeof(float)));
  R2State* st = r2_state((const void*)ot_res2_kernel<false>, nthreads, nblocks, lds);
  if (!st) { set_error("ot_res2_run: no per-device state"); return GIMS_EHIP; }
  if (!st->resident_ok) {
    set_error("the on-chip Sinkhorn kernel does not fit: %d workgroups of %d threads with %zu bytes of LDS are not co-resident on this device", nblocks, nthreads, lds);
    return GIMS_EHIP;
  }
  if (*st->h_place) st->wt_local = 1;
  const int wt_local = st->wt_local;
  int refresh = env_int("GIMS_OT_REFRESH", 0);
  if (refresh == 0 && iters > R2_FLAG_ITERS) refresh = 50;
  const int prof = env_int("GIMS_OT_PROF", 0);
  for (int gi = 0; gi < P.ngroups; ++gi) {
    const int p0 = gi * P.ppg, p1 = (p0 + P.ppg < np) ? p0 + P.ppg : np;
    OtR2Args a{};
    a.probs = dprob; a.p0 = p0; a.pcount = p1 - p0; a.nx = P.nx; a.nc = P.nc; a.alpha = alpha; a.iters = iters; a.refresh = refresh; a.wt_local = wt_local; a.init_inside = init_inside;
    if (prof) {
      unsigned long long* dprof = (unsigned long long*)device_once("ot_res2_prof", 8 * sizeof(unsigned long long), nullptr);
      GIMS_CHECK_ARG(dprof, "ot_res2_run: no profile buffer");
      a.prof = dprof;
      hipLaunchKernelGGL((ot_res2_kernel<true>), dim3(256), dim3(R2_NT), lds, s, a);
      GIMS_LAUNCH_CHECK();
      unsigned long long h[8];
      GIMS_HIP(hipStreamSynchronize(s));
      GIMS_HIP(hipMemcpy(h, dprof, sizeof(h), hipMemcpyDeviceToHost));
      static const char* names[8] = {"derive", "row pass", "publish + wait for the row partials", "fold + publish F", "gather F (incl. wait)", "column pass",
                                     "column edge (incl. wait)", "column update"};
      fprintf(stderr, "[ot_res2 nx=%d nc=%d iters=%d wt=%d] cycles/iteration of workgroup 0:", P.nx, P.nc, iters, wt_local);
      for (int i = 0; i < 8; ++i) fprintf(stderr, "  %s %.0f;", names[i], (double)h[i] / iters);
      fprintf(stderr, "\n");
    } else {
      hipLaunchKernelGGL((ot_res2_kernel<false>), dim3(256), dim3(R2_NT), lds, s, a);
      GIMS_LAUNCH_CHECK();
    }
  }
  if (env_int("GIMS_OT_R2_DEBUG", 0)) {
    int h[4] = {0, 0, 0, 0};
    GIMS_HIP(hipStreamSynchronize(s));
    GIMS_HIP(hipMemcpy(h, dplace, sizeof(h), hipMemcpyDeviceToHost));
    fprintf(stderr, "[ot_res2 debug] nx=%d nc=%d placement flag %d, last bounded wait that ran out: site %d\n", P.nx, P.nc, h[0], h[1]);
  }
  if (!wt_local) {
    if (hipEventQuery(st->place_ev) != hipErrorNotReady) {
      GIMS_HIP(hipMemcpyAsync((void*)st->h_place, dplace, sizeof(int), hipMemcpyDeviceToHost, s));
      GIMS_HIP(hipEventRecord(st->place_ev, s));
    }
  }
  return GIMS_OK;
}

}
```

gims_amd/gmatcher.py:

```python
from __future__ import annotations

import math
import os
import time
import weakref
from typing import Dict, List

import numpy as np
import torch
import torch.nn as nn

from . import hip
from .attention_tiers import MODE_NAMES, AttentionTiers

BN_EPS = 1e-5
LN_EPS = 1e-6


class _Node(nn.Module):
    """Bare container used to reproduce the reference's parameter tree (names only, no forward)."""


def _register(root: nn.Module, dotted: str, tensor: torch.Tensor, buffer: bool):
    mod = root
# ... 429 lines not shown
                    robust=robust, delaunay=delaunay, each=each, norm3_host=norm3_host)

    _edge_cap = 64

    @staticmethod
    def _agc_retry(flags, robust, delaunay=False):
        flags = np.asarray(flags)
        if delaunay:
            bad = np.nonzero(flags & hip.DT_INFO_DEGENERATE)[0]
            if len(bad):
                i = int(bad[0])
                raise ValueError(f"delaunay: image {i} of the batch (pair {i // 2}, keypoints{i % 2}) has fewer than 3 distinct keypoints, "
                                 "all its keypoints on one line, or a non-finite coordinate: it has no Delaunay triangulation")
            if (flags & (hip.DT_INFO_ASYMMETRIC | hip.AGC_INFO_WINDOW_MISSED)).any():
                raise hip.GimsHipError("delaunay graph: the per-point stars of a build did not agree (asymmetric adjacency)")
        if (flags & hip.AGC_INFO_WINDOW_MISSED).any():
            if robust:
                raise hip.GimsHipError("adaptive graph: the robust flow reported a missed percentile window")
            return "robust"
        if (flags & hip.AGC_INFO_OVERFLOW).any():
            return "grow"
        return None

    def _gather(self, ctx):
        images, info_all = ctx["images"], ctx["info_all"]
        cfg = self.config
        dev = images[0]["kp"].device
        D = cfg['descriptor_dim']
        ts0 = time.perf_counter()
        pin = self.__dict__.get("_info_pin")
        if pin is None or pin.shape[0] < info_all.shape[0]:
            pin = self.__dict__["_info_pin"] = torch.empty((max(64, info_all.shape[0]), 8), dtype=torch.int32, pin_memory=True)
        pin[:info_all.shape[0]].copy_(info_all, non_blocking=True)
        early = self._kenc_early(ctx)
        if early is None:
            torch.cuda.current_stream().synchronize()
        else:
            early["event"].synchronize()
        infos = pin[:info_all.shape[0]].numpy().copy()
        self._sync_ms = 1e3 * (time.perf_counter() - ts0)
        each = ctx.get("each")
        if each is None:
            action = self._agc_retry(infos[:, 7], bool(ctx.get("robust")), bool(ctx.get("delaunay")))
        else:
            tri = np.asarray([bool(e[3]) for e in each])
            acts = [self._agc_retry(np.where(tri, infos[:, 7], 0), bool(ctx.get("robust")), True) if tri.any() else None,
                    self._agc_retry(np.where(tri, 0, infos[:, 7]), bool(ctx.get("robust")), False)]
            action = "robust" if "robust" in acts else ("grow" if "grow" in acts else None)
        if action == "robust":
            ctx["params"] = tuple(ctx["params"][:3]) + (True,)
            self._agc_window_misses = getattr(self, "_agc_window_misses", 0) + 1
            return None
        if action == "grow":
            ns = np.asarray([g["kp"].shape[0] for g in images], dtype=np.float64)
            tot = np.maximum(infos[:, 1].astype(np.float64), 2.0 * infos[:, 2] + 2.0 * ns)
            need = int(np.ceil(max(2.0 * self._edge_cap, float((tot / ns).max()) * 1.1)))
            cap = 1 << (need - 1).bit_length()
            if cap > 16384 or cap <= self._edge_cap:
                raise hip.GimsHipError(f"adaptive graph exceeded the edge capacity ({self._edge_cap} directed edges per node) and cannot grow further")
            self._edge_cap = cap
            ctx["params"] = tuple(ctx["params"][:3]) + (bool(ctx.get("robust")),)
            return None
        norm3 = ctx["norm3"]
        if (infos[:, 0] == 0).any():
            if not ctx.get("skip_empty"):
                raise ValueError("need at least one array to concatenate")
            gone = (infos[:, 0].reshape(-1, 2) == 0).any(axis=1)
            ctx["dropped"] = np.nonzero(gone)[0].tolist()
            keep = np.repeat(~gone, 2)
            images = ctx["images"] = [g for g, k in zip(images, keep) if k]
            infos, ctx["ptab"] = infos[keep], ctx["ptab"][keep]
            if not images:
                return dict(n_tot=0)
            norm3 = hip.upload(ctx["norm3_host"][keep], dev)

        row_off = np.concatenate([[0], np.cumsum(infos[:, 0], dtype=np.int64)])
        e_off = np.concatenate([[0], np.cumsum(infos[:, 1], dtype=np.int64)])
        n_tot, e_tot = int(row_off[-1]), int(e_off[-1])
        with GMatcher._Stage(self, "gather"):
            ptab, b = ctx["ptab"], ctx["bufs"]
            ptab["n_kept"], ptab["n_edges"], ptab["row_off"], ptab["edge_off"] = infos[:, 0], infos[:, 1], row_off[:-1], e_off[:-1]
            feat, kpts_all, score_all, seg = b["feat"][:n_tot], b["kpts"][:n_tot], b["score"][:n_tot], b["seg"][:n_tot]
            indptr_all, indices_all = b["indptr"][:n_tot + 1], b["indices"][:max(e_tot, 1)]
            hip.pack_graphs_table(ptab, D, feat, kpts_all, score_all, seg, indptr_all, indices_all, n_tot, e_tot)
        row_off, e_off = row_off.tolist(), e_off.tolist()
        for g, inf, ro in zip(images, infos, row_off):
            g["n_kept"], g["n_edges"], g["info_host"] = int(inf[0]), int(inf[1]), inf
            g["rows"] = (ro, g["n_kept"])
        return dict(feat=feat, kpts_all=kpts_all, score_all=score_all, seg=seg, indptr_all=indptr_all, indices_all=indices_all,
                    norm3=norm3, n_tot=n_tot, e_tot=e_tot, early=early)

    kenc_early = True

    def _kenc_early(self, ctx):
        if not ctx.get("kenc_early") or not self.kenc_early or os.environ.get("GIMS_KENC_EARLY", "1") == "0":
            return None
        images = ctx["images"]
        kp0 = images[0]["kp"]
        dev = kp0.device
        P = self._packed(dev)
        if not P["x3"] or P["ln"]:
            return None
        starts, off = [], 0
        for g in images:
            kp = g["kp"]
            if kp.dtype != torch.float32 or not kp.is_contiguous() or kp.data_ptr() != kp0.data_ptr() + 8 * off:
                return None
            starts.append(off)
            off += kp.shape[0]
        n_in = off
        bf, f32 = torch.bfloat16, torch.float32
        A = lambda name, cols, dt: self._act(name, n_in, cols, dt)
        c1 = P["kenc_w1"].shape[0]
        kmax = max([c1] + [e["n"] for e in P["kenc"]])
        b = dict(xk=A("kenc_in_x", c1, f32), xs0=A("kenc_in_xs0", 2 * kmax, bf), xs1=A("kenc_in_xs1", 2 * kmax, bf), desc=A("kenc_in_out", P["kenc"][-1]["n"], f32))
        src_row = self._act("kenc_src_row", n_in, 1, torch.int32)
        ev = torch.cuda.Event()
        ev.record()
        starts_dev = hip.upload(np.asarray(starts, dtype=np.int32), dev)
        batch = dict(n=n_in, kpts=kp0.data_ptr(), norm3=ctx["norm3"].data_ptr(), seg=starts_dev.data_ptr(), n_img=len(images))
        key = (P["gen"],) + tuple(t.data_ptr() for t in b.values())
        cache = self.__dict__.setdefault("_kenc_cache", {})
        ent = cache.get(key)
        if ent is None:
            if len(cache) > 4:
                cache.clear()
            lst, slots = self._encoder_ops(P, b, None, batch, part="kenc")
            ent = cache[key] = self._table(lst, (P, b), slots)
        self._patch(ent, batch)
        self._issue("encoder", ent, n_in)
        ctx["ptab"]["src_row"], ctx["ptab"]["in_off"] = src_row.data_ptr(), starts
        return dict(event=ev, out=b["desc"], src_row=src_row, starts=starts_dev)

    @staticmethod
    def _patch(ent, batch):
        ops = ent[0]
        for k, field, j, what in ent[6]:
            if j is None:
                setattr(ops[k].u.lin, field, batch[what])
            else:
                getattr(ops[k].u.aux, field)[j] = batch[what]

    @staticmethod
    def _finish_graphs(images, G):
        for g in images:
            ro, nk = g["rows"]
            g["kept"] = g["kept"][:nk]
            g["indptr"] = g["indptr"][:nk + 1]
            g["indices"] = g["indices"][:g["n_edges"]]
            g["graph"] = GraphHandle(g["indptr"], g["indices"],
                                     {"point": G["kpts_all"][ro:ro + nk], "feat": G["feat"][ro:ro + nk], "score": G["score_all"][ro:ro + nk]})

    def _replays(self, part, n_tot):
        if self._stepwise:
            return False
        env = os.environ.get("GIMS_NO_REPLAY")
        if env is not None:
            return env == ("3" if part == "encoder" else "2")
        rows = int(self.config['launch_replay_rows'])
        return os.environ.get("GIMS_REPLAY") == "1" or rows <= 0 or n_tot <= rows

    def _run_rest(self, ctx):
        ctx["kenc_early"] = True
        G = self._gather(ctx)
        if G is None:
            again = self._run_build(ctx["images"], *ctx["params"], delaunay=bool(ctx.get("delaunay")), each=ctx.get("each"))
            again.update({k: ctx[k] for k in ("guards", "repeat", "streamed", "skip_empty") if k in ctx}, repeats=ctx.get("repeats", 0) + 1)
            return self._run_rest(again)
        res = self._last = self._run_batch(ctx, G) if ctx["images"] else dict(items=[], pairs=[], mdesc=None, images=[], outputs=[], status_offs=np.zeros(0, dtype=np.int64))
        res.update(dropped=ctx.get("dropped", []), repeats=ctx.get("repeats", 0))
        return res

    def _run_batch(self, ctx, G):
        images = ctx["images"]
        P = self._packed(images[0]["kp"].device)
        feat, kpts_all, score_all, n_tot = G["feat"], G["kpts_all"], G["score_all"], G["n_tot"]
        sage, desc = self._encoder(P, G)
        pairs = [(images[2 * p]["rows"], images[2 * p + 1]["rows"]) for p in range(len(images) // 2)]
        res = self._match_rows(P, desc, n_tot, pairs, max(g["n_kept"] for g in images), ctx)
        self._finish_graphs(images, G)
        res.update(sage=sage, images=images, outputs=res["outputs"] + [feat, kpts_all, score_all, ctx["pool"]])
        return res

    def _match_rows(self, P, desc, n_tot, pairs, max_nq, ctx):
        cfg = self.config
        dev = desc.device
        D = cfg['descriptor_dim']
        St = lambda name: GMatcher._Stage(self, name)
        spr = np.asarray([[o, n, o, n] for pr in pairs for (o, n) in pr], dtype=np.int32)
        cpr = np.asarray([q for (o0, n0), (o1, n1) in pairs for q in ((o0, n0, o1, n1), (o1, n1, o0, n0))], dtype=np.int32)
        both = hip.upload(np.concatenate([spr, cpr]), dev, out=self._buf("attn_pr", spr.nbytes + cpr.nbytes + 32))
        stat = self._layers(P, desc, n_tot, max_nq, both[:spr.shape[0]], both[spr.shape[0]:], bool(ctx.get("guards")), bool(ctx.get("repeat")))
        if stat is not None:
            self._attention_stats_enqueue(stat)
        with St("final_scores"):
            mdesc = self._lin(P["final"], self._act("dpl", n_tot, 2 * D, torch.bfloat16) if P["x3"] else desc)
            items, largs = [], []
            tot0, tot1 = sum(n0 for (_, n0), _ in pairs), sum(n1 for _, (_, n1) in pairs)
            m0_all = torch.empty(tot0, dtype=torch.int64, device=dev)
            m1_all = torch.empty(tot1, dtype=torch.int64, device=dev)
            s0_all = torch.empty(tot0, dtype=torch.float32, device=dev)
            s1_all = torch.empty(tot1, dtype=torch.float32, device=dev)
            uv_all = torch.empty(tot0 + tot1 + 3 * len(pairs), dtype=torch.float32, device=dev)
            c0 = c1 = cu = 0
            sprec = hip.PREC_BF16X6 if (D % 32 == 0 and os.environ.get("GIMS_SCORE_PREC", "x6") != "f32") else hip.PREC_F32
            sdesc = hip.split_spl3(mdesc) if sprec == hip.PREC_BF16X6 else mdesc
            for (o0, n0), (o1, n1) in pairs:
                ld = (n1 + 3) // 4 * 4
                scores = torch.empty((n0, ld), dtype=torch.float32, device=dev)
                largs.append(hip.linear_args(sdesc[o0:o0 + n0], sdesc[o1:o1 + n1], out=scores, precision=sprec,
                                             scale=1.0 / math.sqrt(D), n=n1))
                items.append(dict(scores=scores, n=n0, m=n1, matches0=m0_all[c0:c0 + n0], matches1=m1_all[c1:c1 + n1],
                                  mscores0=s0_all[c0:c0 + n0], mscores1=s1_all[c1:c1 + n1], uv=uv_all[cu:cu + n0 + n1 + 3]))
                c0, c1, cu = c0 + n0, c1 + n1, cu + n0 + n1 + 3
            hip.linear_batch(largs, self._buf("score_args", 256 * len(largs)), sprec)
        with St("sinkhorn"):
            probs = hip.make_ot_problems(items)
            work = self._buf("ot", hip.sinkhorn_workspace_bytes(probs))
            otf = hip.OT_STREAMED if ctx.get("streamed") else 0
            self.sinkhorn_plan_last = hip.sinkhorn_plan(probs, cfg['sinkhorn_iterations'], otf)
            hip.sinkhorn_match(probs, P["alpha"], cfg['sinkhorn_iterations'], cfg['match_threshold'], work, otf)
            status_offs = np.cumsum([it["n"] + it["m"] + 3 for it in items]) - 1
        return dict(items=items, pairs=pairs, mdesc=mdesc, desc=desc,
                    flat=dict(matches0=m0_all, scores0=s0_all, n0=[n0 for (_, n0), _ in pairs], n1=[n1 for _, (_, n1) in pairs]),
                    outputs=[m0_all, m1_all, s0_all, s1_all, uv_all, mdesc], status_offs=status_offs)

    @staticmethod
    def _lin_op(e, a0, **kw):
        return hip.op_linear(hip.linear_args(a0, e["w"], w_lo=e["w_lo"], bias=e["b"], precision=e["prec"], spl=e["spl"], **kw))

    @staticmethod
    def _norm_args(x, a2b2, rows, out=None, out_split=None):
        return (hip.AUX_LAYERNORM_ACT, [x, a2b2[0], a2b2[1], out, out_split, None if out_split is None else out_split.data_ptr() + 64],
                [x.stride(0), rows, x.shape[1], hip.ACT_RELU, 0 if out is None else out.stride(0), 0 if out_split is None else out_split.stride(0)],
                [LN_EPS])

    @staticmethod
    def _table(lst, keep, *extra):
        runs = []
        for k, (lab, _) in enumerate(lst):
            if runs and runs[-1][0] == lab:
                runs[-1][2] += 1
            else:
                runs.append([lab, k, 1])
        return [hip.make_ops([o for _, o in lst]), None, 0, keep, [lab for lab, _ in lst], runs, *extra]

    def _issue(self, part, ent, n_tot):
        ops, labels, runs = ent[0], ent[4], ent[5]
        if self._replays(part, n_tot) and (part == "layers" or self._timers is None):
            ent[2] += 1
            if (part == "layers" and ent[1] is None and ent[2] >= 2 and self._use_graph
                    and torch.cuda.current_stream().cuda_stream != 0):
                ent[1] = hip.OpsGraph(ops)
            if self._timers is not None:
                pool = hip.EventPool(len(ops) + 1)
                hip.run_ops_timed(ops, pool)
                self._timers.setdefault("_ops", []).append((pool, labels))
            elif ent[1] is not None:
                ent[1].launch()
            else:
                hip.run_ops(ops)
            return
        for label, start, count in runs:
            with GMatcher._Stage(self, label):
                hip.run_ops(ops, start, count)

    def _encoder(self, P, G):
        D, n_tot = self.config['descriptor_dim'], G["n_tot"]
        bf, f32 = torch.bfloat16, torch.float32
        x3, spl = P["x3"], P["x3"] and not P["ln"]
        A = lambda name, cols, dt: self._act(name, n_tot, cols, dt)
        c1 = P["kenc_w1"].shape[0]
        wmax = max([D] + [e["n"] for e in P["sage"]])
        kmax = max([c1] + [e["n"] for e in P["kenc"]])
        early = G.get("early")
        b = dict(hf0=A("sage_h0", wmax, f32), hf1=A("sage_h1", wmax, f32), agg=A("sage_agg", 2 * wmax, bf) if x3 else A("sage_agg", wmax, f32),
                 desc=A("desc", P["kenc"][-1]["n"], f32))
        if early is None:
            b.update(sage=A("sage_out", P["sage"][-1]["n"], f32), xk=A("kenc_x", c1, f32))
        if x3:
            b.update(hs0=A("sage_hs0", 2 * wmax, bf), hs1=A("sage_hs1", 2 * wmax, bf), dpl=A("dpl", 2 * D, bf))
        if early is None and spl:
            b.update(xs0=A("kenc_xs0", 2 * kmax, bf), xs1=A("kenc_xs1", 2 * kmax, bf))
        elif early is None:
            b.update(xf0=A("kenc_xf0", kmax, f32), xf1=A("kenc_xf1", kmax, f32))
        batch = dict(n=n_tot, feat=G["feat"].data_ptr(), ldf=G["feat"].stride(0), indptr=G["indptr_all"].data_ptr(), indices=G["indices_all"].data_ptr(),
                     kpts=G["kpts_all"].data_ptr(), norm3=G["norm3"].data_ptr(), seg=G["seg"].data_ptr())
        if early is not None:
            batch.update(kenc_all=early["out"].data_ptr(), src_row=early["src_row"].data_ptr())
        key = (P["gen"], early is not None) + tuple(t.data_ptr() for t in b.values())
        cache = self.__dict__.setdefault("_enc_cache", {})
        ent = cache.get(key)
        if ent is None:
            if len(cache) > 4:
                cache.clear()
            lst, slots = self._encoder_ops(P, b, G["feat"], batch, part="all" if early is None else "sage", early=early)
            ent = cache[key] = self._table(lst, (P, b), slots)
        self._patch(ent, batch)
        self._issue("encoder", ent, n_tot)
        return b.get("sage"), b["desc"]

    def _encoder_ops(self, P, b, feat, batch, part="all", early=None):
        x3, ln, spl = P["x3"], P["ln"], P["x3"] and not P["ln"]
        lst, slots = [], []
        V = lambda t, cols: t[:, :cols]

        def aux(label, fn, ptrs, ints, floats=()):
            for field, args in (("p", ptrs), ("i", ints)):
                slots.extend((len(lst), field, j, a) for j, a in enumerate(args) if isinstance(a, str))
            lst.append((label, hip.op_aux(fn, [batch[a] if isinstance(a, str) else a for a in ptrs],
                                          [batch[a] if isinstance(a, str) else a for a in ints], floats)))

        def lin(label, e, a0, **kw):
            slots.append((len(lst), "m", None, "n"))
            if kw.get("residual_rows") is not None:
                slots.extend([(len(lst), "residual", None, "kenc_all"), (len(lst), "residual_rows", None, "src_row")])
            if feat is not None and a0 is feat:
                slots.extend([(len(lst), "a0", None, "feat"), (len(lst), "lda0", None, "ldf")])
            lst.append((label, self._lin_op(e, a0, **kw)))
        if part != "kenc":
            self._sage_ops(P, b, feat, aux, lin, V, early)
        if part != "sage":
            self._kenc_ops(P, b, aux, lin, V, part == "kenc")
        return lst, slots

    @staticmethod
    def _sage_ops(P, b, feat, aux, lin, V, early):
        x3 = P["x3"]
        dims = [feat.shape[1]] + [e["n"] for e in P["sage"]]
        h, ldh, hop = "feat", "ldf", feat
        if x3:
            aux("sage", hip.AUX_SPLIT_SPL32, ["feat", b["hs0"]], ["ldf", b["hs0"].stride(0), "n", dims[0]])
            hop = V(b["hs0"], 2 * dims[0])
        for i, e in enumerate(P["sage"]):
            last = i == len(P["sage"]) - 1
            aggv = V(b["agg"], (2 if x3 else 1) * dims[i])
            aux("sage", hip.AUX_SAGE_MEAN_SPLIT if x3 else hip.AUX_SAGE_MEAN, [h, "indptr", "indices", aggv], [ldh, "n", dims[i], aggv.stride(0)])
            if last and early is not None:
                lin("sage", e, hop, a1=aggv, act=hip.ACT_NONE, out=b["desc"], out_split=b.get("dpl"), residual=early["out"], residual_rows=early["src_row"])
                break
            h = b["sage"] if last else V(b["hf%d" % (i & 1)], dims[i + 1])
            hs = V(b["hs%d" % ((i + 1) & 1)], 2 * dims[i + 1]) if x3 and not last else None
            lin("sage", e, hop, a1=aggv, act=hip.ACT_NONE if last else hip.ACT_RELU, out=h, out_split=hs)
            ldh, hop = h.stride(0), hs if x3 else h

    def _kenc_ops(self, P, b, aux, lin, V, images):
        ln, spl = P["ln"], P["x3"] and not P["ln"]
        c1, xk = b["xk"].shape[1], b["xk"]
        aux("kenc", hip.AUX_KENC_FIRST_LINEAR if ln else hip.AUX_KENC_FIRST, ["kpts", "norm3", "seg", P["kenc_w1"], P["kenc_b1"], xk],
            [c1, "n"] + (["n_img"] if images else []))
        if ln:
            aux("kenc", *self._norm_args(xk, P["kenc_ln"][0], "n", out=xk))
        cur = xk
        if spl:
            aux("kenc", hip.AUX_SPLIT_SPL32, [xk, b["xs0"]], [xk.stride(0), b["xs0"].stride(0), "n", c1])
            cur = V(b["xs0"], 2 * c1)
        for i, e in enumerate(P["kenc"]):
            if i == len(P["kenc"]) - 1:
                if images:
                    lin("kenc", e, cur, out=b["desc"])
                else:
                    lin("kenc", e, cur, residual=b["sage"], out=b["desc"], out_split=b.get("dpl"))
            elif spl:
                cur, prev = V(b["xs%d" % ((i + 1) & 1)], 2 * e["n"]), cur
                lin("kenc", e, prev, act=hip.ACT_RELU, out_split=cur)
            else:
                cur, prev = V(b["xf%d" % (i & 1)], e["n"]), cur
                lin("kenc", e, prev, act=hip.ACT_NONE if ln else hip.ACT_RELU, out=cur)
                if ln:
                    aux("kenc", *self._norm_args(cur, P["kenc_ln"][i + 1], "n", out=cur))

    def _layers(self, P, desc, n_tot, max_nq, self_pr, cross_pr, guards, repeat):
        cfg, D = self.config, self.config['descriptor_dim']
        x3 = P["x3"]
        if cfg['attention_precision'] not in ('auto', 'bf16', 'f16', 'bf16x3'):
            raise ValueError("attention_precision must be 'auto', 'bf16', 'f16' or 'bf16x3'")
        if cfg['attention_precision'] in ('f16', 'bf16x3') and not x3:
            raise ValueError(f"attention_precision='{cfg['attention_precision']}' needs linear_precision='bf16x3' (the 3-pass Q/K/V projection)")
        amode, stat = self._attention_modes(P, repeat)
        calibrated = self._tiers is not None and self._tiers.calibrated
        guarded = stat is not None and cfg['attention_precision'] == 'auto' and calibrated and guards
        bf, f32 = torch.bfloat16, torch.float32
        A = lambda name, cols, dt: self._act(name, n_tot, cols, dt)
        one_mlp = self._mlp_fused(P, n_tot)
        self.linear_launches_per_layer = 2 if one_mlp else (3 if cfg['fuse_merge'] else 4)
        b = dict(desc=desc, src=A("dpl", 2 * D, bf) if x3 else desc, stat=stat, self_pr=self_pr, cross_pr=cross_pr,
                 msg=A("mpl", 2 * D, bf) if x3 else A("msg", D, f32), mrg=A("gpl", 2 * D, bf) if x3 else A("mrg", D, f32),
                 hid=None if one_mlp else (A("hpl", 4 * D, bf) if x3 else A("hid", 2 * D, f32)), hid_ln=A("hid_ln", 2 * D, f32) if (x3 and P["ln"]) else None,
                 qkv_b=A("qkv", 3 * D, bf) if not all(a == 2 for a in amode) else None,
                 qkv_s=A("qkv6", 6 * D, bf) if (guarded or any(a == 2 for a in amode)) else None)
        key = (P["gen"], n_tot, max_nq) + tuple(0 if t is None else t.data_ptr() for t in b.values()) + (
            (float(cfg['attention_auto_threshold']), float(cfg['attention_auto_tail']), float(cfg['attention_f16_range']),
             float(cfg['attention_auto_rowmax'])) if guarded else None,
            self_pr.shape[0], cross_pr.shape[0], self._qkv_flags, tuple(amode))
        cache = self.__dict__.setdefault("_ops_cache", {})
        ent = cache.get(key)
        if ent is None:
            if len(cache) > 8:
                cache.clear()
            ent = cache[key] = self._table(self._layer_ops(P, b, n_tot, max_nq, amode, calibrated, guarded), (P, b))
        self._issue("layers", ent, n_tot)
        return stat

    def _layer_ops(self, P, b, n_tot, max_nq, amode, calibrated, guarded):
        cfg, D, H = self.config, self.config['descriptor_dim'], self._heads
        x3, ln, stat = P["x3"], P["ln"], b["stat"]
        desc, src, msg, mrg, hid, qkv_b, qkv_s = b["desc"], b["src"], b["msg"], b["mrg"], b["hid"], b["qkv_b"], b["qkv_s"]
        to = (lambda t: dict(out_split=t)) if x3 else (lambda t: dict(out=t))
        lst = []
        for l, L in enumerate(P["layers"]):
            pr = b["cross_pr"] if L["cross"] else b["self_pr"]
            sfx = ("", "_f16", "_x3")[amode[l]]
            st = None if (stat is None or (calibrated and amode[l] == 2)) else stat[l]
            if amode[l] == 2:
                qkv, qkv_out = qkv_s, dict(out_split=qkv_s)
            elif amode[l] == 1:
                qkv, qkv_out = qkv_b, dict(out_bf16=qkv_b, flags=hip.LINEAR_OUT_F16, range_stat=None if st is None else stat[l][H])
            else:
                qkv, qkv_out = qkv_b, (dict(out_bf16=qkv_b, flags=self._qkv_flags) if x3 else dict(out_bf16=qkv_b))
            lst.append(("qkv" + sfx, self._lin_op(L["qkv"], src, **qkv_out)))
            lst.append((("attn_cross" if L["cross"] else "attn_self") + sfx,
                        hip.op_attention(qkv, pr, max_nq, H, None if x3 else msg, 0, D, 2 * D, out_split=msg if x3 else None, q_prescaled=True,
                                         x3=amode[l] == 2, f16=amode[l] == 1, stat=st, no_range=amode[l] == 1)))
            if guarded and amode[l] != 2:
                gd = (hip.attn_guard(stat[l], hip.GUARD_PEAKED, H, mean_thr=cfg['attention_auto_threshold'], tail_thr=cfg['attention_auto_tail'],
                                     max_thr=cfg['attention_auto_rowmax']) if amode[l] == 0
                      else hip.attn_guard(stat[l], hip.GUARD_RANGE, H, range_limit=cfg['attention_f16_range']))
                lst.append(("guard", self._lin_op(L["qkv"], src, out_split=qkv_s, guard=gd)))
                lst.append(("guard", hip.op_attention(qkv_s, pr, max_nq, H, None, 0, D, 2 * D, out_split=msg, q_prescaled=True, x3=True, guard=gd)))
            m, e0 = msg, L["mlp0_fused"]
            if hid is None:
                lst.append(("mlp", hip.op_mlp(src, msg, L["mlp_op"]["w"], L["mlp_op"]["b"], desc, src, residual=desc)))
                continue
            if e0 is None:
                lst.append(("mlp", self._lin_op(L["merge"], msg, **to(mrg))))
                m, e0 = mrg, L["mlp0"]
            if ln:
                hf = b["hid_ln"] if x3 else hid
# ... 425 lines not shown
```

gims_amd/hip.py:

```python
from __future__ import annotations

import ctypes as C
import math
import os
import threading

import numpy as np
import torch

from . import _abi
from ._abi import GimsHipError

_HERE = os.path.dirname(os.path.abspath(__file__))
LIB_PATH = os.path.join(_HERE, "libgims_hip.so")

ABI = _abi.parse()
_K = ABI.constants
EXPORTS = tuple(ABI.signatures)
ABI_VERSION = _K["GIMS_ABI_VERSION"]
GIMS_OK, GIMS_EINVAL, GIMS_EHIP, GIMS_ENUMERIC = _K["GIMS_OK"], _K["GIMS_EINVAL"], _K["GIMS_EHIP"], _K["GIMS_ENUMERIC"]

PREC_F32, PREC_BF16X3, PREC_BF16X6 = _K["GIMS_PREC_F32"], _K["GIMS_PREC_BF16X3"], _K["GIMS_PREC_BF16X6"]
LINEAR_UPPER = _K["GIMS_LINEAR_UPPER"]
LINEAR_HI_ONLY = _K["GIMS_LINEAR_HI_ONLY"]
LINEAR_OUT_F16 = _K["GIMS_LINEAR_OUT_F16"]
ACT_NONE, ACT_RELU = _K["GIMS_ACT_NONE"], _K["GIMS_ACT_RELU"]

AttnGuard = ABI.structs["gims_attn_guard"]
LinearArgs = ABI.structs["gims_linear_args"]
AttnArgs = ABI.structs["gims_attn_args"]
AuxArgs = ABI.structs["gims_aux_args"]
Op = ABI.structs["gims_op"]
AgcImage = ABI.structs["gims_agc_image"]
AgcParams = ABI.structs["gims_agc_params"]
PackImage = ABI.structs["gims_pack_image"]
IngestImage = ABI.structs["gims_ingest_image"]
OtProblem = ABI.structs["gims_ot_problem"]
PyrLevel = ABI.structs["gims_pyr_level"]
SiftInfo = ABI.structs["gims_sift_info"]
LossPair = ABI.structs["gims_loss_pair"]
Gemm = ABI.structs["gims_gemm"]
TrainAttnProblem = ABI.structs["gims_train_attn_problem"]
TrainAttnArgs = ABI.structs["gims_train_attn_args"]
Segments = ABI.structs["gims_segments"]
AdamTensor = ABI.structs["gims_adam_tensor"]
AdamGroup = ABI.structs["gims_adam_group"]
SgdTensor = ABI.structs["gims_sgd_tensor"]
SgdGroup = ABI.structs["gims_sgd_group"]
EmaTensor = ABI.structs["gims_ema_tensor"]
EvalPair = ABI.structs["gims_eval_pair"]
VerifySet = ABI.structs["gims_verify_set"]
LabelPair = ABI.structs["gims_label_pair"]
NnPair = ABI.structs["gims_nn_pair"]
AugPlan = ABI.structs["gims_aug_plan"]

GUARD_PEAKED, GUARD_RANGE = _K["GIMS_GUARD_PEAKED"], _K["GIMS_GUARD_RANGE"]
AUX_SPLIT_SPL32, AUX_SAGE_MEAN_SPLIT, AUX_KENC_FIRST = _K["GIMS_AUX_SPLIT_SPL32"], _K["GIMS_AUX_SAGE_MEAN_SPLIT"], _K["GIMS_AUX_KENC_FIRST"]
AUX_SAGE_MEAN, AUX_KENC_FIRST_LINEAR, AUX_LAYERNORM_ACT = _K["GIMS_AUX_SAGE_MEAN"], _K["GIMS_AUX_KENC_FIRST_LINEAR"], _K["GIMS_AUX_LAYERNORM_ACT"]
AUX_SIFT_DESCRIBE = _K["GIMS_AUX_SIFT_DESCRIBE"]
AUX_DIOU_NMS = _K["GIMS_AUX_DIOU_NMS"]
AUX_ASSEMBLE_ROWS = _K["GIMS_AUX_ASSEMBLE_ROWS"]
AUX_BUILD_TRACKS = _K["GIMS_AUX_BUILD_TRACKS"]
TRACKS_TABLE_WORDS, TRACKS_KEEP_CONFLICTING = _K["GIMS_TRACKS_TABLE_WORDS"], _K["GIMS_TRACKS_KEEP_CONFLICTING"]
TRACKS_SCAN_TILE = _K["GIMS_TRACKS_SCAN_TILE"]
TRACKS_SHORT_SEGMENT = _K["GIMS_TRACKS_SHORT_SEGMENT"]
TRACKS_LONG_SEGMENT = _K["GIMS_TRACKS_LONG_SEGMENT"]
TRACKS_COUNTERS = ("n_tracks", "n_obs", "n_conflicting", "n_edges", "n_bad", "status")
AUX_TRIANGULATE_TRACKS = _K["GIMS_AUX_TRIANGULATE_TRACKS"]
TRI_CAMERA_WORDS, TRI_MAX_OBS = _K["GIMS_TRI_CAMERA_WORDS"], _K["GIMS_TRI_MAX_OBS"]
TRI_SHORT_TRACK = _K["GIMS_TRI_SHORT_TRACK"]
TRI_COUNTERS = ("n_ok", "n_low_angle", "n_no_model", "n_too_short", "n_too_long", "n_bad_obs", "n_inlier_obs")
TRI_TOO_SHORT, TRI_NO_MODEL, TRI_LOW_ANGLE, TRI_TOO_LONG = 1, 2, 4, 8
AUX_RESECT_IMAGES = _K["GIMS_AUX_RESECT_IMAGES"]
RESECT_CAMERA_WORDS = _K["GIMS_RESECT_CAMERA_WORDS"]
RESECT_HB = _K["GIMS_RESECT_HB"]
RESECT_COUNTERS = ("n_ok", "n_failed", "n_corr_total", "n_inlier_total")
AUX_BUNDLE_ADJUST = _K["GIMS_AUX_BUNDLE_ADJUST"]
BA_TABLE_WORDS, BA_MAX_FREE_CAMERAS, BA_MAX_REJECTS = _K["GIMS_BA_TABLE_WORDS"], _K["GIMS_BA_MAX_FREE_CAMERAS"], _K["GIMS_BA_MAX_REJECTS"]
AUX_BUNDLE_ADJUST_PCG = _K["GIMS_AUX_BUNDLE_ADJUST_PCG"]
BA_PCG_MAX_FREE_CAMERAS, BA_PCG_MAX_CG_ITERS = _K["GIMS_BA_PCG_MAX_FREE_CAMERAS"], _K["GIMS_BA_PCG_MAX_CG_ITERS"]
AUX_BUNDLE_ADJUST_FOCAL = _K["GIMS_AUX_BUNDLE_ADJUST_FOCAL"]
AUX_SELECT_PAIRS = _K["GIMS_AUX_SELECT_PAIRS"]
PAIRS_TABLE_WORDS, PAIRS_SCALE_GIVEN = _K["GIMS_PAIRS_TABLE_WORDS"], _K["GIMS_PAIRS_SCALE_GIVEN"]
PAIRS_MAX_IMAGES, PAIRS_MAX_ROWS, PAIRS_MAX_D = _K["GIMS_PAIRS_MAX_IMAGES"], _K["GIMS_PAIRS_MAX_ROWS"], _K["GIMS_PAIRS_MAX_D"]
PAIRS_QUERY_TILE = _K["GIMS_PAIRS_QUERY_TILE"]
PAIRS_COUNTERS = ("n_pairs", "n_rows", "n_short_images", "n_bad_rows", "n_nonfinite")
BA_COUNTERS = ("n_free", "n_fixed", "n_held", "n_points", "n_active_obs", "n_bad_obs", "rounds_taken", "status")
BA_BAD_CAMERA, BA_BAD_START = 1, 2
BA_ABSENT, BA_FIXED, BA_FREE = 0, 1, 2
SIFT_MAX_OCTAVES, SIFT_MAX_RADIUS, SIFT_SLOTS = _K["GIMS_SIFT_MAX_OCTAVES"], _K["GIMS_SIFT_MAX_RADIUS"], _K["GIMS_SIFT_SLOTS"]


def attn_guard(stat, kind, n_heads, mean_thr=0.0, tail_thr=0.0, range_limit=0.0, max_thr=0.0) -> AttnGuard:
    assert stat.dtype == torch.int64 and stat.is_cuda and stat.is_contiguous() and stat.numel() >= 4 * (n_heads + 1)
    return AttnGuard(stat.data_ptr(), float(mean_thr), float(tail_thr), float(range_limit), int(n_heads), int(kind), float(max_thr))


_lib = None


def load(path: str | None = None):
    global _lib
    if _lib is not None and path is None:
        return _lib
    p = path or LIB_PATH
    if not os.path.exists(p):
        raise GimsHipError(f"{p} is missing: build it with `python -m gims_amd.build` "
                           "(hipcc --offload-arch=gfx950); there is no CPU fallback")
    lib = C.CDLL(p)
    for name, (res, args) in ABI.signatures.items():
        fn = getattr(lib, name)
        fn.restype, fn.argtypes = res, args
    if lib.gims_abi_version() != ABI_VERSION:
        raise GimsHipError(f"ABI version mismatch: library {lib.gims_abi_version()} != binding {ABI_VERSION} (rebuild: python -m gims_amd.build)")
    if path is None:
        _lib = lib
    return lib



def _check(rc: int, what: str):
    if rc != 0:
        msg = load().gims_last_error()
        raise GimsHipError(f"{what} failed ({rc}): {msg.decode() if msg else ''}")


_TLS = threading.local()


def _stream() -> int:
    pin = getattr(_TLS, "pin", None)
    return pin if pin is not None else torch.cuda.current_stream().cuda_stream


class on_stream:

    def __init__(self, handle: int):
        self._h = int(handle)

# ... 341 lines not shown
                              _p(it["kept"]), _p(it["indptr"]), _p(it["indices"]), it["indices"].numel(), _p(it["info"]))
            continue
        assert de.stride(1) == 1
        arr[i] = AgcImage(_p(_dev(it["kpts"], torch.float32)), _p(_dev(de, torch.float32)), de.stride(0), de.shape[0], de.shape[1],
                          _p(it["kept"]), _p(it["indptr"]), _p(it["indices"]), it["indices"].numel(), _p(it["info"]))
    return arr


def agc_max_keypoints() -> int:
    return int(load().gims_agc_max_keypoints())


def agc_workspace_bytes(images, flags=None) -> int:
    nmax = max(int(im.n) for im in images)
    if nmax > agc_max_keypoints():
        raise GimsHipError(f"adaptive graph: an image has {nmax} keypoints, more than the library's limit of {agc_max_keypoints()} per image "
                           "(gims_agc_max_keypoints; the reference has none) -- reduce max_keypoints or split the image")
    return int(load().gims_agc_workspace_bytes(images, len(images), AGC_ROBUST if flags is None else int(flags)))


AGC_ROBUST = _K["GIMS_AGC_ROBUST"]
AGC_INFO_OVERFLOW, AGC_INFO_WINDOW_MISSED = 1, 2


def agc_build(images, radius, percentile, min_size, work: torch.Tensor, flags=0):
    one = AgcParams(float(radius), float(percentile), int(min_size), 0)
    _check(load().gims_agc_build(images, len(images), C.byref(one), 1, int(flags), _p(work), work.numel() * work.element_size(), _stream()),
           "gims_agc_build")


def agc_build_each(images, params, work: torch.Tensor, flags=0):
    params = list(params)
    if len(params) != len(images):
        raise ValueError(f"agc_build_each: {len(images)} images but {len(params)} parameter triples")
    arr = (AgcParams * len(params))(*[AgcParams(float(r), float(t), int(m), 0) for r, t, m in params])
    _check(load().gims_agc_build(images, len(images), arr, len(params), int(flags), _p(work), work.numel() * work.element_size(), _stream()),
           "gims_agc_build")


DT_INFO_DEGENERATE, DT_INFO_ASYMMETRIC = _K["GIMS_DT_INFO_DEGENERATE"], _K["GIMS_DT_INFO_ASYMMETRIC"]


def delaunay_workspace_bytes(images) -> int:
    nmax = max(int(im.n) for im in images)
    if nmax > agc_max_keypoints():
        raise GimsHipError(f"delaunay graph: an image has {nmax} keypoints, more than the library's limit of {agc_max_keypoints()} per image "
                           "(gims_agc_max_keypoints) -- reduce max_keypoints or split the image")
    return int(load().gims_delaunay_workspace_bytes(images, len(images)))


def delaunay_build(images, work: torch.Tensor):
    lib = load()
    _check(lib.gims_delaunay_build(images, len(images), _p(work), work.numel() * work.element_size(), _stream()), "gims_delaunay_build")


def _upload_structs(arr, device):
    nbytes = C.sizeof(arr)
    buf = torch.empty(((nbytes + 15) // 16 * 16 + 16,), dtype=torch.uint8, device=device)
    _check(load().gims_upload_table(C.addressof(arr), nbytes, buf.data_ptr(), _stream()), "gims_upload_table")
    return buf


def ingest_images(items, d, desc_out, kpts_out, score_out):
    lib = load()
    if not any(i.n > 0 for i in items):
        return None
    arr = (IngestImage * len(items))(*items)
    dev_arr = _upload_structs(arr, desc_out.device)
    _check(lib.gims_ingest_images(_p(dev_arr), len(items), max(i.n for i in items), d, _p(desc_out), desc_out.stride(0),
                                  _p(kpts_out), _p(score_out), _stream()), "gims_ingest_images")
    return dev_arr


PACK_DTYPE = np.dtype(PackImage)


def pack_table(images_ptrs):
    t = np.zeros(len(images_ptrs), dtype=PACK_DTYPE)
    for i, r in enumerate(images_ptrs):
        t[i] = tuple(r) + (0,) * (len(PACK_DTYPE.names) - len(r))
    return t


def pack_graphs_table(table, d, feat, kpts_out, score_out, seg, indptr_out, indices_out, n_rows, n_edges):
    lib = load()
    nbytes = table.nbytes
    dev_arr = torch.empty(((nbytes + 15) // 16 * 16 + 16,), dtype=torch.uint8, device=feat.device)
    st = _stream()
    _check(lib.gims_upload_table(table.ctypes.data, nbytes, dev_arr.data_ptr(), st), "gims_upload_table")
    _check(lib.gims_pack_graphs(_p(dev_arr), len(table), int(table["n_kept"].max()), max(int(table["n_edges"].max()), 1), d,
                                _p(feat), feat.stride(0), _p(kpts_out), _p(score_out), _p(seg), _p(indptr_out),
                                _p(indices_out), n_rows, n_edges, st), "gims_pack_graphs")
    return dev_arr


def make_ot_problems(items):
    arr = (OtProblem * len(items))()
    for i, it in enumerate(items):
        s = it["scores"]
        arr[i] = OtProblem(_p(s), s.stride(0), it["n"], it["m"], _p(it["matches0"]), _p(it["matches1"]),
                           _p(it["mscores0"]), _p(it["mscores1"]), _p(it["uv"]))
    return arr


def sinkhorn_workspace_bytes(problems) -> int:
    return int(load().gims_sinkhorn_workspace_bytes(problems, len(problems)))


OT_STREAMED = _K["GIMS_OT_STREAMED"]


def sinkhorn_plan(problems, iters: int, flags: int = 0) -> int:
    return int(load().gims_sinkhorn_plan(problems, len(problems), int(iters), int(flags)))


ATTN_KERNEL_KINDS = ("wave4", "split", "wave8", "wave8_f16", "x3", "x3_guarded")


def attention_launch_counts(reset: bool = False) -> dict:
    buf = (C.c_uint64 * len(ATTN_KERNEL_KINDS))()
    _check(load().gims_attention_launch_counts(buf, len(ATTN_KERNEL_KINDS), int(reset)), "gims_attention_launch_counts")
    return dict(zip(ATTN_KERNEL_KINDS, (int(x) for x in buf)))


LINEAR_KERNEL_NAMES = tuple(k[len("GIMS_LINEAR_KERNEL_"):].lower() for k, _ in sorted(
    ((k, v) for k, v in _K.items() if k.startswith("GIMS_LINEAR_KERNEL_") and k != "GIMS_LINEAR_KERNEL_KINDS"), key=lambda kv: kv[1]))
assert len(LINEAR_KERNEL_NAMES) == _K["GIMS_LINEAR_KERNEL_KINDS"]


def linear_launch_counts(reset: bool = False) -> dict:
    buf = (C.c_uint64 * len(LINEAR_KERNEL_NAMES))()
    _check(load().gims_linear_launch_counts(buf, len(LINEAR_KERNEL_NAMES), int(reset)), "gims_linear_launch_counts")
    return dict(zip(LINEAR_KERNEL_NAMES, (int(x) for x in buf)))


def sinkhorn_rescues() -> int:
    n = int(load().gims_sinkhorn_rescues())
    if n < 0:
        _check(GIMS_EHIP, "gims_sinkhorn_rescues")
    return n


def sinkhorn_match(problems, alpha: float, iters: int, match_threshold: float, work: torch.Tensor, flags: int = 0):
    lib = load()
    _check(lib.gims_sinkhorn_match(problems, len(problems), float(alpha), int(iters), float(match_threshold), _p(work),
                                   work.numel() * work.element_size(), int(flags), _stream()), "gims_sinkhorn_match")


def ot_matrix(scores, n, m, alpha, uv):
    lib = load()
    out = torch.empty((n + 1, m + 1), dtype=torch.float32, device=scores.device)
    _check(lib.gims_ot_matrix(_p(scores), scores.stride(0), n, m, float(alpha), _p(uv), _p(out), _stream()),
           "gims_ot_matrix")
    return out


EVAL_FIELDS = ("n_valid", "n_gt", "n_correct", "n_fn", "precision", "recall", "n_inliers", "err_dlt", "err_ransac", "dlt_ok",
               "ransac_ok")


def eval_pairs(items, dist_thresh=3.0, n_iters=3, ransac_thresh=3.0, ransac_iters=3000, seed=0, work=None):
    lib = load()
    arr = (EvalPair * len(items))()
    for i, it in enumerate(items):
        k0, k1 = it["kpts0"], it["kpts1"]
        assert k0.dtype == torch.float32 and k1.dtype == torch.float32 and k0.is_contiguous() and k1.is_contiguous()
        assert it["matches0"].dtype == torch.int64 and it["mscores0"].dtype == torch.float32
        assert it["gt0"].dtype == torch.int32 and it["inlier"].dtype == torch.uint8
        h = np.asarray(it["h_gt"], dtype=np.float32).reshape(9)
        arr[i] = EvalPair(_p(k0), _p(k1), _p(it["matches0"]), _p(it["mscores0"]), k0.shape[0], k1.shape[0], int(it["height"]),
                          int(it["width"]), (C.c_float * 9)(*h.tolist()), _p(it["gt0"]), _p(it["inlier"]), _p(it["record"]),
                          _p(it["homographies"]))
    need = int(lib.gims_eval_workspace_bytes(arr, len(items), int(ransac_iters)))
# ... 1126 lines not shown
```

include/gims_hip.h:

```cpp
#ifndef GIMS_HIP_H
#define GIMS_HIP_H

#include <stddef.h>
#include <stdint.h>

#ifdef __cplusplus
extern "C" {
#endif

#define GIMS_ABI_VERSION 4

#define GIMS_OK 0
#define GIMS_EINVAL (-1)
#define GIMS_EHIP (-2)
#define GIMS_ENUMERIC (-3)

int gims_abi_version(void);
const char* gims_last_error(void);
int gims_upload_table(const void* host, int64_t bytes, void* dev, void* stream);

#define GIMS_PREC_F32 0
#define GIMS_PREC_BF16X3 1
#define GIMS_PREC_BF16X6 2
#define GIMS_ACT_NONE 0
// ... 106 lines not shown
#define GIMS_TRACKS_SHORT_SEGMENT 32
#define GIMS_TRACKS_LONG_SEGMENT 1024
#define GIMS_TRACKS_KEEP_CONFLICTING (1 << 30)
#define GIMS_AUX_TRIANGULATE_TRACKS 10
#define GIMS_TRI_CAMERA_WORDS 18
#define GIMS_TRI_MAX_OBS 1024
#define GIMS_TRI_SHORT_TRACK 4
#define GIMS_AUX_RESECT_IMAGES 11
#define GIMS_RESECT_CAMERA_WORDS 6
#define GIMS_RESECT_HB 16
#define GIMS_AUX_BUNDLE_ADJUST 13
#define GIMS_BA_TABLE_WORDS 8
#define GIMS_BA_MAX_FREE_CAMERAS 128
#define GIMS_BA_MAX_REJECTS 5
#define GIMS_AUX_BUNDLE_ADJUST_PCG 14
#define GIMS_BA_PCG_MAX_FREE_CAMERAS 65536
#define GIMS_BA_PCG_MAX_CG_ITERS 256
#define GIMS_AUX_BUNDLE_ADJUST_FOCAL 16
#define GIMS_AUX_SELECT_PAIRS 17
#define GIMS_PAIRS_TABLE_WORDS 8
#define GIMS_PAIRS_MAX_IMAGES 8192
#define GIMS_PAIRS_MAX_ROWS 4096
#define GIMS_PAIRS_MAX_D 1024
#define GIMS_PAIRS_QUERY_TILE 128
#define GIMS_PAIRS_SCALE_GIVEN 1
typedef struct gims_aux_args { int32_t fn, reserved; const void* p[6]; int64_t i[6]; float f[2]; } gims_aux_args;
typedef struct gims_op { int32_t kind; int32_t reserved; union { gims_linear_args lin; gims_attn_args att; gims_aux_args aux; } u; } gims_op;
int gims_run_ops(const gims_op* ops , int32_t n_ops, void* stream);
int gims_run_ops_timed(const gims_op* ops , int32_t n_ops, void* stream, void* const* events );
int gims_events_create(int32_t n, void** events_out );
int gims_events_elapsed(void* const* events , int32_t n, float* h_ms_out );
int gims_events_destroy(void* const* events , int32_t n);
int gims_ops_graph_create(const gims_op* ops , int32_t n_ops, void* stream, void** graph_exec_out);
int gims_ops_graph_launch(void* graph_exec, void* stream);
int gims_ops_graph_destroy(void* graph_exec);

int gims_kenc_first(const float* kpts, const float* norm3 , const int32_t* seg_of_row,
                    const float* w1, const float* b1, int32_t c1, float* out, int64_t n, void* stream);
int gims_kenc_first_linear(const float* kpts, const float* norm3, const int32_t* seg_of_row,
                           const float* w1, const float* b1, int32_t c1, float* out, int64_t n, void* stream);

int gims_layernorm_act(const float* x, int64_t ldx, int64_t rows, int32_t c, const float* a2, const float* b2, float eps,
                       int32_t act, float* out , int64_t ldo, uint16_t* out_hi ,
                       uint16_t* out_lo, int64_t ld_split, void* stream);

int gims_sage_mean(const float* h, int64_t ldh, const int32_t* indptr, const int32_t* indices,
                   int32_t n, int32_t c, float* out, int64_t ldo, void* stream);
int gims_sage_mean_split(const float* h, int64_t ldh, const int32_t* indptr, const int32_t* indices,
                         int32_t n, int32_t c, uint16_t* out_spl, int64_t ld_spl, void* stream);

int gims_pair_stats(const int64_t* matches0, const float* scores0, const int32_t* table, int32_t n_pairs, float* out, void* stream);

int gims_gather_rows(const float* src, int64_t lds, const int32_t* idx, int32_t n, int32_t c,
                     float* dst, int64_t ldd, void* stream);

typedef struct gims_agc_image {
  const float* kpts; const float* desc; int64_t ldd; int32_t n, d;
  int32_t* kept; int32_t* indptr; int32_t* indices; int32_t max_edges_dir; int32_t* info;
} gims_agc_image;

#define GIMS_AGC_ROBUST 1
size_t gims_agc_workspace_bytes(const gims_agc_image* h_images , int32_t n_images, int32_t flags);
int32_t gims_agc_max_keypoints(void);
typedef struct gims_agc_params { double radius, percentile; int32_t min_size, reserved; } gims_agc_params;
int gims_agc_build(const gims_agc_image* h_images , int32_t n_images, const gims_agc_params* h_params ,
                   int32_t n_params, int32_t flags, void* work, size_t work_bytes, void* stream);

#define GIMS_DT_INFO_DEGENERATE 4
#define GIMS_DT_INFO_ASYMMETRIC 8
size_t gims_delaunay_workspace_bytes(const gims_agc_image* h_images , int32_t n_images);
int gims_delaunay_build(const gims_agc_image* h_images , int32_t n_images, void* work, size_t work_bytes, void* stream);

typedef struct gims_ingest_image {
  const float* kpts; const float* desc; int64_t ldd; const float* score; int32_t n, row_off;
} gims_ingest_image;

int gims_ingest_images(const gims_ingest_image* dev_images , int32_t n_images, int32_t max_n, int32_t d,
                       float* desc_out, int64_t ldo, float* kpts_out, float* score_out , void* stream);

typedef struct gims_pack_image {
  const float* kpts; const float* desc; int64_t ldd; const float* score;
  const int32_t* kept; const int32_t* indptr; const int32_t* indices;
  int32_t n_kept, n_edges, row_off, edge_off;
  int32_t* src_row; int32_t in_off, reserved;
} gims_pack_image;

int gims_pack_graphs(const gims_pack_image* dev_images , int32_t n_images, int32_t max_kept,
                     int32_t max_edges, int32_t d, float* feat, int64_t ldf, float* kpts_out, float* score_out,
                     int32_t* seg, int32_t* indptr_out, int32_t* indices_out, int32_t n_rows_total,
                     int32_t n_edges_total, void* stream);

typedef struct gims_ot_problem {
  const float* scores; int64_t ld; int32_t n, m;
  int64_t* matches0; int64_t* matches1; float* mscores0; float* mscores1;
  float* uv;
} gims_ot_problem;

size_t gims_sinkhorn_workspace_bytes(const gims_ot_problem* h_problems, int32_t n_problems);
#define GIMS_OT_STREAMED 1
int gims_sinkhorn_plan(const gims_ot_problem* h_problems, int32_t n_problems, int32_t iters, int32_t flags);
int gims_sinkhorn_match(const gims_ot_problem* h_problems , int32_t n_problems, float alpha,
                        int32_t iters, float match_threshold, void* work, size_t work_bytes, int32_t flags, void* stream);

int64_t gims_sinkhorn_rescues(void);

typedef struct gims_eval_pair {
  const float* kpts0; const float* kpts1;
  const int64_t* matches0;
  const float* mscores0;
  int32_t n0, n1, height, width;
  float h_gt[9];
  int32_t* gt0; uint8_t* inlier; float* record; float* homographies;
} gims_eval_pair;
#define GIMS_EVAL_NVALID 0
#define GIMS_EVAL_NGT 1
#define GIMS_EVAL_NCORRECT 2
#define GIMS_EVAL_NFN 3
#define GIMS_EVAL_PRECISION 4
#define GIMS_EVAL_RECALL 5
#define GIMS_EVAL_NINLIERS 6
#define GIMS_EVAL_ERR_DLT 7
#define GIMS_EVAL_ERR_RANSAC 8
#define GIMS_EVAL_DLT_OK 9
#define GIMS_EVAL_RANSAC_OK 10
size_t gims_eval_workspace_bytes(const gims_eval_pair* h_pairs, int32_t n_pairs, int32_t ransac_iters);
int gims_eval_pairs(const gims_eval_pair* h_pairs , int32_t n_pairs, float dist_thresh, int32_t n_iters,
                    float ransac_thresh, int32_t ransac_iters, uint64_t seed, void* work, size_t work_bytes, void* stream);

#define GIMS_VERIFY_MODEL_HOMOGRAPHY 0
#define GIMS_VERIFY_MODEL_FUNDAMENTAL 1
#define GIMS_VERIFY_MODEL_POSE 3
typedef struct gims_verify_set {
  const float* kpts0; const float* kpts1;
  const int64_t* matches0;
  int32_t n0, n1, height, width;
  int32_t has_ref, model;
  float h_ref[9];
  uint8_t* inlier; float* record; float* homography;
} gims_verify_set;
#define GIMS_VERIFY_NVALID 0
#define GIMS_VERIFY_OK 1
#define GIMS_VERIFY_NINLIERS 2
#define GIMS_VERIFY_BEST_HYP 3
#define GIMS_VERIFY_BEST_HYP_INLIERS 4
#define GIMS_VERIFY_LO_ROUNDS 5
#define GIMS_VERIFY_ERR_CORNER 6
size_t gims_verify_workspace_bytes(const gims_verify_set* h_sets, int32_t n_sets, int32_t iters);
int gims_verify_pairs(const gims_verify_set* h_sets , int32_t n_sets, float thresh, int32_t iters, int32_t lo_iters,
                      uint64_t seed, void* work, size_t work_bytes, void* stream);

int gims_ot_matrix(const float* scores, int64_t ld, int32_t n, int32_t m, float alpha, const float* uv,
                   float* out , void* stream);

typedef struct gims_loss_pair {
  const float* scores; int64_t ld; int32_t n, m; const float* uv; const int32_t* kept0; const int32_t* kept1;
} gims_loss_pair;
int gims_train_loss(const gims_loss_pair* dev_pairs , int32_t n_pairs, const int64_t* gt, int32_t n_gt, float alpha,
                    float pos_weight, float neg_weight, float* loss_vec, int32_t* tag, float* out3, void* stream);

size_t gims_sinkhorn_history_floats(int32_t n, int32_t m, int32_t iters);
int gims_sinkhorn_history(const gims_ot_problem* h_problems, int32_t n_problems, float alpha, int32_t iters, float* const* h_hist ,
                          void* work , size_t work_bytes, void* stream);
size_t gims_sinkhorn_backward_workspace_bytes(const gims_ot_problem* h_problems, int32_t n_problems);
int gims_sinkhorn_backward(const gims_ot_problem* h_problems, int32_t n_problems, float alpha, int32_t iters, const float* const* h_hist ,
                           float* const* h_dz , float* dalpha , void* work, size_t work_bytes, void* stream);
int gims_train_loss_grad(const gims_loss_pair* dev_pairs, int32_t n_pairs, const int64_t* gt, int32_t n_gt, float alpha, const int32_t* tag,
                         float pos_weight, float neg_weight, float* const* dev_dz_ptrs , void* stream);

// ... 160 lines not shown
```

Baseline: 571.0 pairs/s.

## Fold small launches into producer kernels across AGC, packing, encoder and Sinkhorn

Folds the AGC finish kernel into the final fill kernel. Has graph packing and the first keypoint-encoder layer write the bf16 hi/lo split planes directly, removing separate split kernels. Replaces the Sinkhorn on-chip setup memsets, table upload and status-zero kernel with one prep kernel that carries the problem records as kernel arguments. The aim is fewer tiny launches and memory passes per step, at the cost of more complex producer kernels and env-gated dual paths.

```diff
diff --git a/gims_amd/csrc/agc.hip b/gims_amd/csrc/agc.hip
--- a/gims_amd/csrc/agc.hip
+++ b/gims_amd/csrc/agc.hip
@@ -1011,8 +1011,11 @@
   }
 }
 
-__global__ __launch_bounds__(256) void agc_fill_kernel(const AgcWs* __restrict__ ws, int final_pass) {
-  const AgcWs& w = ws[blockIdx.y];
+__device__ __forceinline__ void agc_finish_body(const AgcWs& w, int window);
+
+__global__ __launch_bounds__(256) void agc_fill_kernel(const AgcWs* __restrict__ ws, int final_pass, int finish) {
+  const AgcWs& w = ws[blockIdx.y];
+  if (finish && blockIdx.x == 0 && threadIdx.x == 0) agc_finish_body(w, finish - 1);
   const int32_t* __restrict__ ptr_by_row = final_pass ? w.indptr : w.ptr0;
   const int32_t* __restrict__ newid = final_pass ? w.newid : nullptr;
   int32_t* __restrict__ idx = final_pass ? w.indices : w.idx0;
@@ -1299,8 +1302,8 @@
   if (added) atomicAdd(&info[5], added);
 }
 
-__global__ void agc_finish_kernel(const AgcWs* __restrict__ ws, int window) {
-  const AgcWs& w = ws[blockIdx.y];
+__global__ void agc_finish_kernel(const AgcWs* __restrict__ ws, int window) { agc_finish_body(ws[blockIdx.y], window); }
+__device__ __forceinline__ void agc_finish_body(const AgcWs& w, int window) {
   int32_t* info = w.info;
   const int max_edges_dir = w.max_edges_dir;
   info[2] = w.counters[0] / 2;
@@ -1404,6 +1407,7 @@
   const bool robust = agc_takes_robust_flow(images, n_images, flags);
   const char* env_shift = getenv("GIMS_AGC_WINDOW_SHIFT");
   const float window_test_shift = env_shift ? (float)atof(env_shift) : 0.f;
+  const int fold = env_int("GIMS_AGC_FOLD", 1) != 0 ? 1 : 0;
   for (int i = 0; i < n_images; ++i) {
     const gims_agc_image& im = images[i];
     GIMS_CHECK_ARG(im.kpts && im.desc && im.kept && im.indptr && im.indices && im.info, "gims_agc_build: image %d has a null pointer", i);
@@ -1487,7 +1491,7 @@
   hipLaunchKernelGGL(agc_iso_seq_kernel, g1, dim3(1024), iso_lds, s, dws);
   hipLaunchKernelGGL(agc_deg_kernel, dim3(cdiv(maxn, 16), B), dim3(256), 0, s, dws, 0);
   hipLaunchKernelGGL(agc_scan_kernel, g1, dim3(1024), 0, s, dws, 0);
-  hipLaunchKernelGGL(agc_fill_kernel, dim3(cdiv(maxn, 16), B), dim3(256), 0, s, dws, 0);
+  hipLaunchKernelGGL(agc_fill_kernel, dim3(cdiv(maxn, 16), B), dim3(256), 0, s, dws, 0, 0);
   if (maxn <= AGC_CC_LDS_N) hipLaunchKernelGGL(agc_cc_kernel<false>, g1, dim3(1024), (size_t)maxn * 8, s, dws);
   else hipLaunchKernelGGL(agc_cc_kernel<true>, g1, dim3(1024), 0, s, dws);
   hipLaunchKernelGGL(agc_scan_kernel, g1, dim3(1024), 0, s, dws, 1);
@@ -1499,8 +1503,8 @@
   hipLaunchKernelGGL(agc_deg_kernel, dim3(cdiv(maxn, 16), B), dim3(256), 0, s, dws, 0);
   hipLaunchKernelGGL(agc_kept_deg_kernel, dim3(cdiv(maxn, 256), B), dim3(256), 0, s, dws);
   hipLaunchKernelGGL(agc_scan_kernel, g1, dim3(1024), 0, s, dws, 2);
-  hipLaunchKernelGGL(agc_fill_kernel, dim3(cdiv(maxn, 16), B), dim3(256), 0, s, dws, 1);
-  hipLaunchKernelGGL(agc_finish_kernel, g1, dim3(1), 0, s, dws, robust ? 0 : 1);
+  hipLaunchKernelGGL(agc_fill_kernel, dim3(cdiv(maxn, 16), B), dim3(256), 0, s, dws, 1, fold ? (robust ? 1 : 2) : 0);
+  if (!fold) hipLaunchKernelGGL(agc_finish_kernel, g1, dim3(1), 0, s, dws, robust ? 0 : 1);
   GIMS_LAUNCH_CHECK();
   return GIMS_OK;
 }
diff --git a/gims_amd/csrc/common.h b/gims_amd/csrc/common.h
--- a/gims_amd/csrc/common.h
+++ b/gims_amd/csrc/common.h
@@ -154,6 +154,7 @@
 struct OtR2Host { const float* z; int64_t ld; int n, m; float* u; float* v; float* status; float norm, log_mu_bin, log_nu_bin; };
 struct OtR2Plan { bool ok; int nx, nc, ppg, ngroups; size_t bytes; };
 OtR2Plan ot_res2_plan(const OtR2Host* pr, int np, int iters);
-int ot_res2_run(const OtR2Plan& P, const OtR2Host* hp, int np, float alpha, int iters, int init_inside, char* base, hipStream_t s);
+int ot_res2_run(const OtR2Plan& P, const OtR2Host* hp, int np, float alpha, int iters, int init_inside, int zero_status, char* base, hipStream_t s);
+static inline bool ot_prep_enabled() { return env_int("GIMS_OT_PREP", 1) != 0; }
 
 }
diff --git a/gims_amd/csrc/misc.hip b/gims_amd/csrc/misc.hip
--- a/gims_amd/csrc/misc.hip
+++ b/gims_amd/csrc/misc.hip
@@ -101,7 +101,7 @@
 __global__ __launch_bounds__(256) void kenc_first_kernel(const float* __restrict__ kpts, const float* __restrict__ norm3,
                                                          const int32_t* __restrict__ seg, const float* __restrict__ w1,
                                                          const float* __restrict__ b1, int c1, float* __restrict__ out,
-                                                         int64_t n, int n_img) {
+                                                         int64_t n, int n_img, uint16_t* __restrict__ out_spl, int64_t ld_spl) {
   const int64_t idx = (int64_t)blockIdx.x * blockDim.x + threadIdx.x;
   const int64_t row = idx / c1;
   const int ch = (int)(idx - row * c1);
@@ -121,7 +121,13 @@
   const float x = (kpts[2 * row] - nm[0]) / nm[2];
   const float y = (kpts[2 * row + 1] - nm[1]) / nm[2];
   float v = fmaf(w1[2 * ch + 1], y, fmaf(w1[2 * ch], x, b1[ch]));
-  out[row * c1 + ch] = RELU ? fmaxf(v, 0.f) : v;
+  v = RELU ? fmaxf(v, 0.f) : v;
+  out[row * c1 + ch] = v;
+  if (out_spl) {
+    const uint16_t h = f2bf(v);
+    out_spl[row * ld_spl + spl_col(ch)] = h;
+    out_spl[row * ld_spl + spl_col(ch) + 32] = f2bf(v - bf2f(h));
+  }
 }
 
 __global__ __launch_bounds__(256) void layernorm_act_kernel(const float* __restrict__ x, int64_t ldx, int64_t rows, int c,
@@ -234,11 +240,25 @@
                                                           int n_edges_total) {
   const gims_pack_image im = imgs[blockIdx.y];
   const int wave = threadIdx.x >> 6, lane = threadIdx.x & 63;
+  uint16_t* feat_spl = nullptr;
+  int64_t ld_spl = 0;
+  if (imgs[0].reserved == GIMS_PACK_SPLIT) { feat_spl = (uint16_t*)imgs[gridDim.y].desc; ld_spl = imgs[gridDim.y].ldd; }
   for (int r = blockIdx.x * 4 + wave; r < im.n_kept; r += gridDim.x * 4) {
     const int src = im.kept[r];
     const float4* s = (const float4*)(im.desc + (int64_t)src * im.ldd);
     float4* o = (float4*)(feat + (int64_t)(im.row_off + r) * ldf);
-    for (int q = lane; 4 * q < d; q += 64) o[q] = s[q];
+    for (int q = lane; 4 * q < d; q += 64) {
+      const float4 x = s[q];
+      o[q] = x;
+      if (feat_spl) {
+        const uint32_t h01 = pack_bf2(x.x, x.y), h23 = pack_bf2(x.z, x.w);
+        const uint32_t l01 = pack_bf2(x.x - __uint_as_float(h01 << 16), x.y - __uint_as_float(h01 & 0xffff0000u));
+        const uint32_t l23 = pack_bf2(x.z - __uint_as_float(h23 << 16), x.w - __uint_as_float(h23 & 0xffff0000u));
+        uint16_t* os = feat_spl + (int64_t)(im.row_off + r) * ld_spl + spl_col(4 * q);
+        *(uint2*)os = make_uint2(h01, h23);
+        *(uint2*)(os + 32) = make_uint2(l01, l23);
+      }
+    }
     if (lane == 0) {
       kpts_out[2 * (im.row_off + r)] = im.kpts[2 * src];
       kpts_out[2 * (im.row_off + r) + 1] = im.kpts[2 * src + 1];
@@ -314,12 +334,13 @@
   return GIMS_OK;
 }
 
-static int kenc_first_images(const float* kpts, const float* norm3, const int32_t* starts, const float* w1, const float* b1, int32_t c1,
-                             float* out, int64_t n, int32_t n_img, hipStream_t stream) {
-  using namespace gims;
-  GIMS_CHECK_ARG(kpts && norm3 && starts && w1 && b1 && out && c1 > 0 && n >= 0, "gims_run_ops: GIMS_AUX_KENC_FIRST: bad arguments");
+static int kenc_first_table(const float* kpts, const float* norm3, const int32_t* starts, const float* w1, const float* b1, int32_t c1,
+                            float* out, int64_t n, int32_t n_img, uint16_t* out_spl, int64_t ld_spl, hipStream_t stream) {
+  using namespace gims;
+  GIMS_CHECK_ARG(kpts && norm3 && starts && w1 && b1 && out && c1 > 0 && n >= 0 && n_img >= 0, "gims_run_ops: GIMS_AUX_KENC_FIRST: bad arguments");
+  GIMS_CHECK_ARG(!out_spl || ((c1 % 32) == 0 && ld_spl >= 2 * (int64_t)c1), "gims_run_ops: GIMS_AUX_KENC_FIRST: split output needs c1 %% 32 == 0 and a pitch >= 2 c1");
   if (n == 0) return GIMS_OK;
-  hipLaunchKernelGGL(kenc_first_kernel<true>, dim3(cdiv(n * c1, 256)), dim3(256), 0, stream, kpts, norm3, starts, w1, b1, c1, out, n, n_img);
+  hipLaunchKernelGGL(kenc_first_kernel<true>, dim3(cdiv(n * c1, 256)), dim3(256), 0, stream, kpts, norm3, starts, w1, b1, c1, out, n, n_img, out_spl, ld_spl);
   GIMS_LAUNCH_CHECK();
   return GIMS_OK;
 }
@@ -342,9 +363,9 @@
       else if (x.fn == GIMS_AUX_SAGE_MEAN_SPLIT)
         rc = gims_sage_mean_split((const float*)x.p[0], x.i[0], (const int32_t*)x.p[1], (const int32_t*)x.p[2], (int32_t)x.i[1], (int32_t)x.i[2],
                                   (uint16_t*)x.p[3], x.i[3], stream);
-      else if (x.fn == GIMS_AUX_KENC_FIRST && x.i[2] > 0)
-        rc = kenc_first_images((const float*)x.p[0], (const float*)x.p[1], (const int32_t*)x.p[2], (const float*)x.p[3], (const float*)x.p[4],
-                               (int32_t)x.i[0], (float*)x.p[5], x.i[1], (int32_t)x.i[2], (hipStream_t)stream);
+      else if (x.fn == GIMS_AUX_KENC_FIRST && (x.i[2] > 0 || x.i[3] != 0))
+        rc = kenc_first_table((const float*)x.p[0], (const float*)x.p[1], (const int32_t*)x.p[2], (const float*)x.p[3], (const float*)x.p[4],
+                              (int32_t)x.i[0], (float*)x.p[5], x.i[1], (int32_t)x.i[2], (uint16_t*)(uintptr_t)x.i[3], x.i[4], (hipStream_t)stream);
       else if (x.fn == GIMS_AUX_KENC_FIRST)
         rc = gims_kenc_first((const float*)x.p[0], (const float*)x.p[1], (const int32_t*)x.p[2], (const float*)x.p[3], (const float*)x.p[4],
                              (int32_t)x.i[0], (float*)x.p[5], x.i[1], stream);
@@ -469,7 +490,7 @@
   GIMS_CHECK_ARG(kpts && norm3 && seg_of_row && w1 && b1 && out && c1 > 0 && n >= 0, "gims_kenc_first: bad arguments");
   if (n == 0) return GIMS_OK;
   hipLaunchKernelGGL(kenc_first_kernel<true>, dim3(cdiv(n * c1, 256)), dim3(256), 0, (hipStream_t)stream, kpts, norm3,
-                     seg_of_row, w1, b1, c1, out, n, 0);
+                     seg_of_row, w1, b1, c1, out, n, 0, (uint16_t*)nullptr, (int64_t)0);
   GIMS_LAUNCH_CHECK();
   return GIMS_OK;
 }
@@ -480,7 +501,7 @@
   GIMS_CHECK_ARG(kpts && norm3 && seg_of_row && w1 && b1 && out && c1 > 0 && n >= 0, "gims_kenc_first_linear: bad arguments");
   if (n == 0) return GIMS_OK;
   hipLaunchKernelGGL(kenc_first_kernel<false>, dim3(cdiv(n * c1, 256)), dim3(256), 0, (hipStream_t)stream, kpts, norm3,
-                     seg_of_row, w1, b1, c1, out, n, 0);
+                     seg_of_row, w1, b1, c1, out, n, 0, (uint16_t*)nullptr, (int64_t)0);
   GIMS_LAUNCH_CHECK();
   return GIMS_OK;
 }
diff --git a/gims_amd/csrc/sinkhorn.hip b/gims_amd/csrc/sinkhorn.hip
--- a/gims_amd/csrc/sinkhorn.hip
+++ b/gims_amd/csrc/sinkhorn.hip
@@ -1129,8 +1129,9 @@
   const OtDev* dp = (const OtDev*)work;
   const bool onchip = w.plan2.ok && iters >= 1;
   const int init_inside = onchip && env_int("GIMS_OT_R2_INIT", 1) ? 1 : 0;
-  if (init_inside) hipLaunchKernelGGL(ot_status0_kernel, dim3(cdiv(np, 256)), dim3(256), 0, s, dp, np);
-  else hipLaunchKernelGGL(ot_init_kernel, dim3(cdiv(maxn, 4), np), dim3(256), 0, s, dp, alpha, iters == 0 ? 1 : 0, 0);
+  const int status_in_prep = init_inside && ot_prep_enabled() ? 1 : 0;
+  if (init_inside && !status_in_prep) hipLaunchKernelGGL(ot_status0_kernel, dim3(cdiv(np, 256)), dim3(256), 0, s, dp, np);
+  else if (!init_inside) hipLaunchKernelGGL(ot_init_kernel, dim3(cdiv(maxn, 4), np), dim3(256), 0, s, dp, alpha, iters == 0 ? 1 : 0, 0);
   const dim3 gi(w.maxG, np);
   if (onchip) {
     std::vector<OtR2Host> h2(np);
@@ -1138,7 +1139,7 @@
       const OtDev& d = hprob[i];
       h2[i] = OtR2Host{d.z, d.ld, d.n, d.m, d.u, d.v, d.status, d.norm, d.log_mu_bin, d.log_nu_bin};
     }
-    const int rc = ot_res2_run(w.plan2, h2.data(), np, alpha, iters, init_inside, w.onchip, s);
+    const int rc = ot_res2_run(w.plan2, h2.data(), np, alpha, iters, init_inside, status_in_prep, w.onchip, s);
     if (rc != GIMS_OK) return rc;
     const int force_fail = env_int("GIMS_OT_FORCE_FAIL", 0);
     if (force_fail) hipLaunchKernelGGL(ot_poison_kernel, dim3(np), dim3(256), 0, s, dp);
diff --git a/gims_amd/csrc/sinkhorn2d.hip b/gims_amd/csrc/sinkhorn2d.hip
--- a/gims_amd/csrc/sinkhorn2d.hip
+++ b/gims_amd/csrc/sinkhorn2d.hip
@@ -1,6 +1,7 @@
 #include "common.h"
 
 #include <stdlib.h>
+#include <string.h>
 
 #include <map>
 #include <mutex>
@@ -835,7 +836,7 @@
   return P;
 }
 
-static int run_class(const OtR2Plan& P, const OtR2Host* hp, int np, float alpha, int iters, int init_inside, char* base, hipStream_t s);
+static int run_class(const OtR2Plan& P, const OtR2Host* hp, int np, float alpha, int iters, int init_inside, int zero_status, char* base, hipStream_t s);
 
 struct R2State { int resident_ok, wt_local; volatile int* h_place; hipEvent_t place_ev; };
 static R2State* r2_state(const void* kernel, int threads, int blocks, size_t lds) {
@@ -856,30 +857,65 @@
   return &states.emplace(dev, st).first->second;
 }
 
-int ot_res2_run(const OtR2Plan&, const OtR2Host* hp, int np, float alpha, int iters, int init_inside, char* base, hipStream_t s) {
+int ot_res2_run(const OtR2Plan&, const OtR2Host* hp, int np, float alpha, int iters, int init_inside, int zero_status, char* base, hipStream_t s) {
   WsLayout L(base);
   for (const std::vector<int>& cls : r2_classes(hp, np)) {
     std::vector<OtR2Host> sub;
     for (int i : cls) sub.push_back(hp[i]);
     const OtR2Plan c = plan_class(sub.data(), (int)sub.size(), iters);
     if (!c.ok) { set_error("ot_res2_run: a geometry class has no plan"); return GIMS_EINVAL; }
-    const int rc = run_class(c, sub.data(), (int)sub.size(), alpha, iters, init_inside, L.take<char>(c.bytes), s);
+    const int rc = run_class(c, sub.data(), (int)sub.size(), alpha, iters, init_inside, zero_status, L.take<char>(c.bytes), s);
     if (rc != GIMS_OK) return rc;
   }
   return GIMS_OK;
 }
 
-static int run_class(const OtR2Plan& P, const OtR2Host* hp, int np, float alpha, int iters, int init_inside, char* base, hipStream_t s) {
+constexpr int R2_PREP_RECS = 3968 / (int)sizeof(OtR2Dev);
+struct R2PrepTable { OtR2Dev rec[R2_PREP_RECS]; };
+__global__ __launch_bounds__(256) void r2_prep_kernel(R2PrepTable tab, int in_args, OtR2Dev* dprob, int np, int zero_status, uint4* __restrict__ fill,
+                                                       int64_t n_ff0, int64_t n_ff1, int64_t n_all) {
+  if (blockIdx.x == 0) {
+    for (int i = threadIdx.x; i < np; i += 256) {
+      float* status;
+      if (in_args) { dprob[i] = tab.rec[i]; status = tab.rec[i].status; }
+      else status = dprob[i].status;
+      if (zero_status) status[0] = 0.f;
+    }
+  }
+  const uint4 ff = make_uint4(0xffffffffu, 0xffffffffu, 0xffffffffu, 0xffffffffu), zero = make_uint4(0u, 0u, 0u, 0u);
+  for (int64_t i = (int64_t)blockIdx.x * 256 + threadIdx.x; i < n_all; i += (int64_t)gridDim.x * 256) fill[i] = (i >= n_ff0 && i < n_ff1) ? ff : zero;
+}
+
+static int run_class(const OtR2Plan& P, const OtR2Host* hp, int np, float alpha, int iters, int init_inside, int zero_status, char* base, hipStream_t s) {
   std::vector<OtR2Dev> hd(np);
   WsLayout L(base);
   const R2Ws w = r2_layout(P, hp, np, L, hd.data());
   OtR2Dev* const dprob = w.dprob;
   int* const dplace = w.dplace;
-  GIMS_HIP(hipMemsetAsync(base + w.ex0, 0xFF, w.ex1 - w.ex0, s));
-  GIMS_HIP(hipMemsetAsync(base + w.ex1, 0, w.rf1 - w.ex1, s));
-  GIMS_HIP(hipMemsetAsync(dplace, 0, 256, s));
-  int rc = upload_table(hd.data(), sizeof(OtR2Dev) * (size_t)np, dprob, s);
-  if (rc != GIMS_OK) return rc;
+  static_assert(sizeof(R2PrepTable) <= 3968 && R2_PREP_RECS <= 256, "the records of r2_prep_kernel are kernel arguments, one per thread of its first workgroup");
+  if (ot_prep_enabled()) {
+    GIMS_CHECK_ARG((char*)dplace + 256 == base + w.ex0 && w.ex0 <= w.ex1 && w.ex1 <= w.rf1 && (w.ex0 % 16) == 0, "ot_res2_run: unexpected workspace layout");
+    R2PrepTable tab;
+    memset(&tab, 0, sizeof(tab));
+    const int in_args = np <= R2_PREP_RECS ? 1 : 0;
+    if (in_args) memcpy(tab.rec, hd.data(), sizeof(OtR2Dev) * (size_t)np);
+    else {
+      const int rc = upload_table(hd.data(), sizeof(OtR2Dev) * (size_t)np, dprob, s);
+      if (rc != GIMS_OK) return rc;
+    }
+    const int64_t n_ff0 = 16, n_ff1 = n_ff0 + (int64_t)((w.ex1 - w.ex0) / 16), n_all = n_ff0 + (int64_t)((w.rf1 - w.ex0) / 16);
+    int grid = (int)((n_all + 1023) / 1024);
+    grid = grid < 1 ? 1 : (grid > 2048 ? 2048 : grid);
+    hipLaunchKernelGGL(r2_prep_kernel, dim3(grid), dim3(256), 0, s, tab, in_args, dprob, np, zero_status, (uint4*)dplace, n_ff0, n_ff1, n_all);
+    GIMS_LAUNCH_CHECK();
+  } else {
+    GIMS_HIP(hipMemsetAsync(base + w.ex0, 0xFF, w.ex1 - w.ex0, s));
+    GIMS_HIP(hipMemsetAsync(base + w.ex1, 0, w.rf1 - w.ex1, s));
+    GIMS_HIP(hipMemsetAsync(dplace, 0, 256, s));
+    const int rc = upload_table(hd.data(), sizeof(OtR2Dev) * (size_t)np, dprob, s);
+    if (rc != GIMS_OK) return rc;
+  }
+  int rc = GIMS_OK;
   const int nthreads = R2_NT, nblocks = 256;
   const size_t lds = R2L::FLOATS * sizeof(float);
   GIMS_LDS_ATTR((const void*)ot_res2_kernel<false>, (int)(R2L::FLOATS * sizeof(float)));
diff --git a/gims_amd/gmatcher.py b/gims_amd/gmatcher.py
--- a/gims_amd/gmatcher.py
+++ b/gims_amd/gmatcher.py
@@ -535,13 +535,26 @@
             ptab["n_kept"], ptab["n_edges"], ptab["row_off"], ptab["edge_off"] = infos[:, 0], infos[:, 1], row_off[:-1], e_off[:-1]
             feat, kpts_all, score_all, seg = b["feat"][:n_tot], b["kpts"][:n_tot], b["score"][:n_tot], b["seg"][:n_tot]
             indptr_all, indices_all = b["indptr"][:n_tot + 1], b["indices"][:max(e_tot, 1)]
-            hip.pack_graphs_table(ptab, D, feat, kpts_all, score_all, seg, indptr_all, indices_all, n_tot, e_tot)
+            feat_spl = self._feat_planes(dev, n_tot)
+            hip.pack_graphs_table(ptab, D, feat, kpts_all, score_all, seg, indptr_all, indices_all, n_tot, e_tot, feat_spl=feat_spl)
         row_off, e_off = row_off.tolist(), e_off.tolist()
         for g, inf, ro in zip(images, infos, row_off):
             g["n_kept"], g["n_edges"], g["info_host"] = int(inf[0]), int(inf[1]), inf
             g["rows"] = (ro, g["n_kept"])
         return dict(feat=feat, kpts_all=kpts_all, score_all=score_all, seg=seg, indptr_all=indptr_all, indices_all=indices_all,
-                    norm3=norm3, n_tot=n_tot, e_tot=e_tot, early=early)
+                    norm3=norm3, n_tot=n_tot, e_tot=e_tot, early=early, feat_spl=feat_spl is not None)
+
+    def _feat_planes(self, dev, n_tot):
+        P = self._packed(dev)
+        D = self.config['descriptor_dim']
+        if not P["x3"] or D % 32 or not self._split_at_producer():
+            return None
+        wmax = max([D] + [e["n"] for e in P["sage"]])
+        return self._act("sage_hs0", n_tot, 2 * wmax, torch.bfloat16)
+
+    @staticmethod
+    def _split_at_producer():
+        return os.environ.get("GIMS_PACK_SPLIT", "1") != "0"
 
     kenc_early = True
 
@@ -572,13 +585,14 @@
         ev.record()
         starts_dev = hip.upload(np.asarray(starts, dtype=np.int32), dev)
         batch = dict(n=n_in, kpts=kp0.data_ptr(), norm3=ctx["norm3"].data_ptr(), seg=starts_dev.data_ptr(), n_img=len(images))
-        key = (P["gen"],) + tuple(t.data_ptr() for t in b.values())
+        kenc_spl = self._split_at_producer()
+        key = (P["gen"], kenc_spl) + tuple(t.data_ptr() for t in b.values())
         cache = self.__dict__.setdefault("_kenc_cache", {})
         ent = cache.get(key)
         if ent is None:
             if len(cache) > 4:
                 cache.clear()
-            lst, slots = self._encoder_ops(P, b, None, batch, part="kenc")
+            lst, slots = self._encoder_ops(P, b, None, batch, part="kenc", kenc_spl=kenc_spl)
             ent = cache[key] = self._table(lst, (P, b), slots)
         self._patch(ent, batch)
         self._issue("encoder", ent, n_in)
@@ -741,19 +755,21 @@
                      kpts=G["kpts_all"].data_ptr(), norm3=G["norm3"].data_ptr(), seg=G["seg"].data_ptr())
         if early is not None:
             batch.update(kenc_all=early["out"].data_ptr(), src_row=early["src_row"].data_ptr())
-        key = (P["gen"], early is not None) + tuple(t.data_ptr() for t in b.values())
+        feat_spl, kenc_spl = bool(G.get("feat_spl")), self._split_at_producer()
+        key = (P["gen"], early is not None, feat_spl, kenc_spl) + tuple(t.data_ptr() for t in b.values())
         cache = self.__dict__.setdefault("_enc_cache", {})
         ent = cache.get(key)
         if ent is None:
             if len(cache) > 4:
                 cache.clear()
-            lst, slots = self._encoder_ops(P, b, G["feat"], batch, part="all" if early is None else "sage", early=early)
+            lst, slots = self._encoder_ops(P, b, G["feat"], batch, part="all" if early is None else "sage", early=early, feat_spl=feat_spl,
+                                           kenc_spl=kenc_spl)
             ent = cache[key] = self._table(lst, (P, b), slots)
         self._patch(ent, batch)
         self._issue("encoder", ent, n_tot)
         return b.get("sage"), b["desc"]
 
-    def _encoder_ops(self, P, b, feat, batch, part="all", early=None):
+    def _encoder_ops(self, P, b, feat, batch, part="all", early=None, feat_spl=False, kenc_spl=False):
         x3, ln, spl = P["x3"], P["ln"], P["x3"] and not P["ln"]
         lst, slots = [], []
         V = lambda t, cols: t[:, :cols]
@@ -772,18 +788,19 @@
                 slots.extend([(len(lst), "a0", None, "feat"), (len(lst), "lda0", None, "ldf")])
             lst.append((label, self._lin_op(e, a0, **kw)))
         if part != "kenc":
-            self._sage_ops(P, b, feat, aux, lin, V, early)
+            self._sage_ops(P, b, feat, aux, lin, V, early, feat_spl)
         if part != "sage":
-            self._kenc_ops(P, b, aux, lin, V, part == "kenc")
+            self._kenc_ops(P, b, aux, lin, V, part == "kenc", kenc_spl)
         return lst, slots
 
     @staticmethod
-    def _sage_ops(P, b, feat, aux, lin, V, early):
+    def _sage_ops(P, b, feat, aux, lin, V, early, feat_spl=False):
         x3 = P["x3"]
         dims = [feat.shape[1]] + [e["n"] for e in P["sage"]]
         h, ldh, hop = "feat", "ldf", feat
         if x3:
-            aux("sage", hip.AUX_SPLIT_SPL32, ["feat", b["hs0"]], ["ldf", b["hs0"].stride(0), "n", dims[0]])
+            if not feat_spl:
+                aux("sage", hip.AUX_SPLIT_SPL32, ["feat", b["hs0"]], ["ldf", b["hs0"].stride(0), "n", dims[0]])
             hop = V(b["hs0"], 2 * dims[0])
         for i, e in enumerate(P["sage"]):
             last = i == len(P["sage"]) - 1
@@ -797,16 +814,18 @@
             lin("sage", e, hop, a1=aggv, act=hip.ACT_NONE if last else hip.ACT_RELU, out=h, out_split=hs)
             ldh, hop = h.stride(0), hs if x3 else h
 
-    def _kenc_ops(self, P, b, aux, lin, V, images):
+    def _kenc_ops(self, P, b, aux, lin, V, images, kenc_spl=False):
         ln, spl = P["ln"], P["x3"] and not P["ln"]
         c1, xk = b["xk"].shape[1], b["xk"]
+        kenc_spl = kenc_spl and spl and c1 % 32 == 0
         aux("kenc", hip.AUX_KENC_FIRST_LINEAR if ln else hip.AUX_KENC_FIRST, ["kpts", "norm3", "seg", P["kenc_w1"], P["kenc_b1"], xk],
-            [c1, "n"] + (["n_img"] if images else []))
+            [c1, "n"] + (["n_img"] if images else [0] if kenc_spl else []) + ([b["xs0"].data_ptr(), b["xs0"].stride(0)] if kenc_spl else []))
         if ln:
             aux("kenc", *self._norm_args(xk, P["kenc_ln"][0], "n", out=xk))
         cur = xk
         if spl:
-            aux("kenc", hip.AUX_SPLIT_SPL32, [xk, b["xs0"]], [xk.stride(0), b["xs0"].stride(0), "n", c1])
+            if not kenc_spl:
+                aux("kenc", hip.AUX_SPLIT_SPL32, [xk, b["xs0"]], [xk.stride(0), b["xs0"].stride(0), "n", c1])
             cur = V(b["xs0"], 2 * c1)
         for i, e in enumerate(P["kenc"]):
             if i == len(P["kenc"]) - 1:
diff --git a/gims_amd/hip.py b/gims_amd/hip.py
--- a/gims_amd/hip.py
+++ b/gims_amd/hip.py
@@ -55,6 +55,7 @@
 AugPlan = ABI.structs["gims_aug_plan"]
 
 GUARD_PEAKED, GUARD_RANGE = _K["GIMS_GUARD_PEAKED"], _K["GIMS_GUARD_RANGE"]
+PACK_SPLIT = _K["GIMS_PACK_SPLIT"]
 AUX_SPLIT_SPL32, AUX_SAGE_MEAN_SPLIT, AUX_KENC_FIRST = _K["GIMS_AUX_SPLIT_SPL32"], _K["GIMS_AUX_SAGE_MEAN_SPLIT"], _K["GIMS_AUX_KENC_FIRST"]
 AUX_SAGE_MEAN, AUX_KENC_FIRST_LINEAR, AUX_LAYERNORM_ACT = _K["GIMS_AUX_SAGE_MEAN"], _K["GIMS_AUX_KENC_FIRST_LINEAR"], _K["GIMS_AUX_LAYERNORM_ACT"]
 AUX_SIFT_DESCRIBE = _K["GIMS_AUX_SIFT_DESCRIBE"]
@@ -562,13 +563,21 @@
     return t
 
 
-def pack_graphs_table(table, d, feat, kpts_out, score_out, seg, indptr_out, indices_out, n_rows, n_edges):
-    lib = load()
+def pack_graphs_table(table, d, feat, kpts_out, score_out, seg, indptr_out, indices_out, n_rows, n_edges, feat_spl=None):
+    lib = load()
+    n_images = len(table)
+    if feat_spl is not None:
+        if d % 32 or feat_spl.dtype != torch.bfloat16 or feat_spl.stride(1) != 1 or feat_spl.stride(0) < 2 * d or feat_spl.stride(0) % 4 \
+                or feat_spl.shape[0] < n_rows or feat_spl.data_ptr() % 8:
+            raise ValueError("pack_graphs_table: feat_spl must be bf16 [n_rows, >= 2 d] with d a multiple of 32")
+        table = np.concatenate([table, np.zeros(1, dtype=table.dtype)])
+        table["reserved"][0] = PACK_SPLIT
+        table["desc"][n_images], table["ldd"][n_images] = feat_spl.data_ptr(), feat_spl.stride(0)
     nbytes = table.nbytes
     dev_arr = torch.empty(((nbytes + 15) // 16 * 16 + 16,), dtype=torch.uint8, device=feat.device)
     st = _stream()
     _check(lib.gims_upload_table(table.ctypes.data, nbytes, dev_arr.data_ptr(), st), "gims_upload_table")
-    _check(lib.gims_pack_graphs(_p(dev_arr), len(table), int(table["n_kept"].max()), max(int(table["n_edges"].max()), 1), d,
+    _check(lib.gims_pack_graphs(_p(dev_arr), n_images, int(table["n_kept"].max()), max(int(table["n_edges"].max()), 1), d,
                                 _p(feat), feat.stride(0), _p(kpts_out), _p(score_out), _p(seg), _p(indptr_out),
                                 _p(indices_out), n_rows, n_edges, st), "gims_pack_graphs")
     return dev_arr
diff --git a/include/gims_hip.h b/include/gims_hip.h
--- a/include/gims_hip.h
+++ b/include/gims_hip.h
@@ -212,8 +212,10 @@
   const float* kpts; const float* desc; int64_t ldd; const float* score;
   const int32_t* kept; const int32_t* indptr; const int32_t* indices;
   int32_t n_kept, n_edges, row_off, edge_off;
-  int32_t* src_row; int32_t in_off, reserved;
+  int32_t* src_row; int32_t in_off;
+  int32_t reserved;
 } gims_pack_image;
+#define GIMS_PACK_SPLIT 1
 
 int gims_pack_graphs(const gims_pack_image* dev_images , int32_t n_images, int32_t max_kept,
                      int32_t max_edges, int32_t d, float* feat, int64_t ldf, float* kpts_out, float* score_out,
```

New measurement: 570.8 pairs/s. Within noise of the previous version (-0.0%).
